# grantjr1842/index-tts

Measured on AMD Instinct MI355X. Metric: synthesised audio seconds per second (IndexTTS-2 infer_v2 hot path), whole job, higher is better.
Workload: dtype f32 (greedy decode + its prefill: exact fp32 MFMA; fp32 accumulate and fp32 activations everywhere) + split-bf16 (fp32 operands as hi+lo bf16, 3 bf16 MFMAs per product) GEMMs, DiT attention and convolutions in s2mel, the latent pass and the vocoder; GPT linear weights STORED as bf16 (rounded once at

## Files before the change

index-tts_amd/csrc/capi.hip:

```cpp
#include <cstring>
#include <new>

#include "../../include/idxtts.h"
#include "bigvgan.h"
#include "cond.h"
#include "semantic.h"
#include "codec.h"
#include "audio.h"
#include "campplus.h"
#include "conv1d.h"
#include "ctx.h"
#include "gpt.h"
#include "model_util.h"
#include "s2mel.h"

namespace idxtts {

static thread_local std::string g_last_error;

void set_error(const std::string& msg) { g_last_error = msg; }
int fail(const char* file, int line, const std::string& msg) {
  const char* base = std::strrchr(file, '/');
  g_last_error = std::string(base ? base + 1 : file) + ":" + std::to_string(line) + ": " + msg;
  return 1;
}

int aa_act_forward(void* y, const void* x, const float* up_f, const float* down_f, const float* log_alpha,
                   const float* log_beta, int B, int C, int T, hipStream_t stream, const int* lens = nullptr, int len_mul = 1, int dtype = 0);

}

using namespace idxtts;

struct idxtts_conv1d {
  ConvWeights w;
  DeviceArena arena;
  int Cout = 0;
};

struct idxtts_linear {
  LinearWeights w;
  DeviceArena arena;
};

#define API_BEGIN try {
#define API_END                                                        \
  }                                                                    \
  catch (const std::exception& e) { return fail(__FILE__, __LINE__, std::string("exception: ") + e.what()); } \
  catch (...) { return fail(__FILE__, __LINE__, "unknown exception"); }

extern "C" {

int idxtts_version(void) { return 100; }

const char* idxtts_last_error(void) { return g_last_error.c_str(); }

int idxtts_aa_act_fwd(void* out, const void* in, const float* up_filter, const float* down_filter,
                      const float* log_alpha, const float* log_beta, int B, int C, int T, int dtype, void* stream) {
  API_BEGIN
  IDX_CHECK(dtype == IDXTTS_DTYPE_F32 || dtype == IDXTTS_DTYPE_F16 || dtype == IDXTTS_DTYPE_BF16, "dtype must be IDXTTS_DTYPE_F32 / F16 / BF16");
  IDX_CHECK(B >= 0 && C >= 0 && T >= 0, "negative shape");
  return aa_act_forward(out, in, up_filter, down_filter, log_alpha, log_beta, B, C, T, static_cast<hipStream_t>(stream), nullptr, 1, dtype);
  API_END
}

static int fetch(const float* src, size_t n, std::vector<float>* dst) {
  dst->resize(n);
  if (!n) return 0;
  const hipError_t e = hipMemcpy(dst->data(), src, n * sizeof(float), hipMemcpyDefault);
  if (e == hipErrorNoDevice) {
    (void)hipGetLastError();
    memcpy(dst->data(), src, n * sizeof(float));
    return 0;
  }
  IDX_HIP(e);
  return 0;
}

int idxtts_conv1d_create(const float* weight, const float* bias, int Cout, int Cin, int K, int transposed_stride,
                         idxtts_conv1d** out) {
  API_BEGIN
  IDX_CHECK(weight && out, "null pointer");
  IDX_CHECK(Cout > 0 && Cin > 0 && K > 0 && transposed_stride >= 1, "bad shape");
  std::unique_ptr<idxtts_conv1d> c(new idxtts_conv1d());
  std::vector<float> hw, hb;
  if (fetch(weight, (size_t)Cout * Cin * K, &hw)) return 1;
  c->Cout = Cout;
  c->w.Cin = Cin;
  c->w.nchunk = cdiv(Cin, CONV_KC);
  c->w.ups = transposed_stride;
  if (transposed_stride > 1) {
    IDX_CHECK(K == 2 * transposed_stride, "ConvTranspose1d kernel must be 2*stride");
    c->w.M = Cout * transposed_stride;
    c->w.K = 3;
  } else {
    c->w.M = Cout;
    c->w.K = K;
  }
  std::vector<float> packed(conv_packed_floats(c->w.M, Cin, c->w.K));
  if (transposed_stride > 1) pack_conv_transpose1d(packed.data(), hw.data(), Cin, Cout, K, transposed_stride);
  else pack_conv1d(packed.data(), hw.data(), Cout, Cin, K);
  float* d = nullptr;
  if (c->arena.upload(packed.data(), packed.size(), &d)) return 1;
  c->w.wp = d;
  {
    std::vector<float> p16(packed.size());
    pack_conv_bf16x3(p16.data(), packed.data(), packed.size() / CONV_SUB);
    if (c->arena.upload(p16.data(), p16.size(), &d)) return 1;
    c->w.wp16 = d;
  }
  if (bias) {
    if (fetch(bias, Cout, &hb)) return 1;
    if (c->arena.upload(hb.data(), hb.size(), &d)) return 1;
    c->w.bias = d;
  }
  *out = c.release();
  return 0;
  API_END
}

int idxtts_conv1d_fwd(const idxtts_conv1d* conv, const float* x, float* y, const float* residual, int B, int T,
                      int dilation, int pad_left, int pad_mode, float scale, int accumulate, void* stream) {
  API_BEGIN
  IDX_CHECK(conv, "null handle");
  if (B == 0 || T == 0) return 0;
  ConvArgs a;
  a.x = x; a.y = y; a.res = residual; a.B = B; a.T = T; a.dil = dilation; a.pad_left = pad_left;
  a.pad_mode = pad_mode; a.scale = scale; a.accum = accumulate;
  return conv1d_forward(conv->w, a, static_cast<hipStream_t>(stream));
  API_END
}

int idxtts_conv1d_destroy(idxtts_conv1d* conv) {
  delete conv;
  return 0;
}

int idxtts_ctx_load_tensor(idxtts_ctx* ctx, const char* name, const float* data, const int64_t* shape, int ndim) {
  API_BEGIN
  IDX_CHECK(ctx && name && shape, "null pointer");
  IDX_CHECK(!ctx->finalized, "context already finalized");
  IDX_CHECK(ndim >= 0 && ndim <= 8, "ndim");
  const std::string key(name);
  if (!ctx->model->accepts(key)) IDX_FAIL("unknown tensor name '" + key + "'");
  HostTensor t;
  t.shape.assign(shape, shape + ndim);
  const int64_t n = t.numel();
  IDX_CHECK(n >= 0, "negative numel");
  IDX_CHECK(n == 0 || data, "null data");
  if (fetch(data, (size_t)n, &t.data)) return 1;
  ctx->tensors[key] = std::move(t);
  return 0;
  API_END
}

int idxtts_ctx_finalize(idxtts_ctx* ctx) {
  API_BEGIN
  IDX_CHECK(ctx, "null ctx");
  IDX_CHECK(!ctx->finalized, "context already finalized");
  if (ctx->model->finalize(ctx->tensors, ctx->arena)) return 1;
  ctx->tensors.clear();
  ctx->finalized = true;
  return 0;
  API_END
}

int idxtts_ctx_get_tensor(idxtts_ctx* ctx, const char* name, float* host_out, size_t capacity) {
  API_BEGIN
  IDX_CHECK(ctx && name && host_out, "null pointer");
  IDX_CHECK(!ctx->finalized, "staged tensors are released by finalize");
  auto it = ctx->tensors.find(name);
  if (it == ctx->tensors.end()) IDX_FAIL(std::string("no staged tensor '") + name + "'");
  IDX_CHECK(capacity >= it->second.data.size(), "output buffer too small");
  std::copy(it->second.data.begin(), it->second.data.end(), host_out);
  return 0;
  API_END
}

int idxtts_ctx_destroy(idxtts_ctx* ctx) {
  delete ctx;
  return 0;
}

float idxtts_fp8_e4m3_decode(unsigned char code) { return fp8_e4m3_decode(code); }
unsigned char idxtts_fp8_e4m3_encode(float v) { return fp8_e4m3_encode(v); }

int idxtts_bigvgan_create(const idxtts_bigvgan_config* cfg, idxtts_ctx** out) {
  API_BEGIN
  IDX_CHECK(cfg && out, "null pointer");
  std::unique_ptr<idxtts_ctx> ctx(new idxtts_ctx());
  ctx->model.reset(new BigVGANModel(*cfg));
  *out = ctx.release();
  return 0;
  API_END
}

size_t idxtts_bigvgan_workspace_bytes(const idxtts_ctx* ctx, int B, int Tm) {
  if (!ctx || B <= 0 || Tm <= 0) return 0;
  auto* m = dynamic_cast<const BigVGANModel*>(ctx->model.get());
  return m ? m->workspace_bytes(B, Tm) : 0;
}

int idxtts_bigvgan_fwd(idxtts_ctx* ctx, const float* mel, float* wav, int B, int Tm, void* workspace,
                       size_t workspace_bytes, int clamp, int stage_idx, float* stage_out, void* stream) {
  API_BEGIN
  IDX_CHECK(ctx, "null ctx");
  IDX_CHECK(ctx->finalized, "context not finalized");
  auto* m = dynamic_cast<BigVGANModel*>(ctx->model.get());
  IDX_CHECK(m, "not a BigVGAN context");
  IDX_CHECK(B >= 0 && Tm >= 0, "negative shape");
  return m->forward(mel, wav, B, Tm, workspace, workspace_bytes, clamp, stage_idx, stage_out, static_cast<hipStream_t>(stream));
  API_END
}

int idxtts_bigvgan_fwd_ragged(idxtts_ctx* ctx, const float* mel, const int* mel_lengths, float* wav, int B, int Tm, void* workspace,
                              size_t workspace_bytes, int clamp, void* stream) {
  API_BEGIN
  IDX_CHECK(ctx && ctx->finalized, "context not finalized");
  auto* m = dynamic_cast<BigVGANModel*>(ctx->model.get());
  IDX_CHECK(m, "not a BigVGAN context");
  IDX_CHECK(B >= 0 && Tm >= 0 && mel_lengths, "shape / lengths");
  return m->forward(mel, wav, B, Tm, workspace, workspace_bytes, clamp, 0, nullptr, static_cast<hipStream_t>(stream), mel_lengths);
  API_END
}


int idxtts_linear_create(const float* weight, const float* bias, int N, int K, int weight_is_kn, idxtts_linear** out) {
  API_BEGIN
  IDX_CHECK(weight && out && N > 0 && K > 0, "bad arguments");
  std::unique_ptr<idxtts_linear> l(new idxtts_linear());
  std::vector<float> hw, hb;
  if (fetch(weight, (size_t)N * K, &hw)) return 1;
  if (bias && fetch(bias, N, &hb)) return 1;
  if (make_linear(l->arena, hw.data(), bias ? hb.data() : nullptr, N, K, {WP16_ALWAYS, weight_is_kn ? W_KN : W_NK}, &l->w)) return 1;
  *out = l.release();
  return 0;
  API_END
}

int idxtts_linear_fwd(const idxtts_linear* lin, const float* x, int ldx, float* y, int ldy, const float* residual, int ldr, int M,
                      int act, int bf16x3, void* stream) {
  API_BEGIN
  IDX_CHECK(lin, "null handle");
  GemmArgs a;
  a.x = x; a.ldx = ldx; a.y = y; a.ldy = ldy; a.res = residual; a.ldr = ldr; a.M = M; a.act = act;
  return bf16x3 ? gemm_bf16x3_forward(lin->w, a, static_cast<hipStream_t>(stream)) : gemm_tn_forward(lin->w, a, static_cast<hipStream_t>(stream));
  API_END
}

int idxtts_linear_destroy(idxtts_linear* lin) {
  delete lin;
  return 0;
}

int idxtts_attention_fwd(const float* q, const float* k, const float* v, float* o, long q_batch_stride, int q_token_stride,
                         long kv_batch_stride, int kv_token_stride, long o_batch_stride, int o_token_stride, int B, int H,
                         int Sq, int Sk, int causal, const int* kstart, const int* kend, float scale, void* stream) {
  API_BEGIN
  AttnArgs a;
  a.q = q; a.k = k; a.v = v; a.o = o;
  a.q_bs = q_batch_stride; a.k_bs = a.v_bs = kv_batch_stride; a.o_bs = o_batch_stride;
  a.q_ts = q_token_stride; a.k_ts = a.v_ts = kv_token_stride; a.o_ts = o_token_stride;
  a.B = B; a.H = H; a.Sq = Sq; a.Sk = Sk; a.causal = causal; a.kstart = kstart; a.kend = kend; a.scale = scale;
  return flash_attn_forward(a, static_cast<hipStream_t>(stream));
  API_END
}

int idxtts_attention_relkey_fwd(const float* q, const float* k, const float* v, float* o, long batch_stride, int token_stride,
                                long o_batch_stride, int o_token_stride, int B, int H, int S, const int* kend, float scale,
                                const float* rel_key, int rel_left, int rel_right, int split_bf16, void* stream) {
  API_BEGIN
  IDX_CHECK(rel_key, "rel_key is null");
  AttnArgs a;
  a.q = q; a.k = k; a.v = v; a.o = o;
  a.q_bs = a.k_bs = a.v_bs = batch_stride; a.o_bs = o_batch_stride;
  a.q_ts = a.k_ts = a.v_ts = token_stride; a.o_ts = o_token_stride;
  a.B = B; a.H = H; a.Sq = S; a.Sk = S; a.causal = 0; a.kend = kend; a.scale = scale;
  a.rel_key = rel_key; a.rel_left = rel_left; a.rel_right = rel_right; a.split_bf16 = split_bf16 ? 1 : 0;
  return flash_attn_forward(a, static_cast<hipStream_t>(stream));
  API_END
}

int idxtts_attention_bf16x3_fwd(const float* q, const float* k, const float* v, float* o, long q_batch_stride, int q_token_stride,
                         long kv_batch_stride, int kv_token_stride, long o_batch_stride, int o_token_stride, int B, int H,
                         int Sq, int Sk, int causal, const int* kstart, const int* kend, float scale, void* stream) {
  API_BEGIN
  AttnArgs a;
  a.q = q; a.k = k; a.v = v; a.o = o;
  a.q_bs = q_batch_stride; a.k_bs = a.v_bs = kv_batch_stride; a.o_bs = o_batch_stride;
  a.q_ts = q_token_stride; a.k_ts = a.v_ts = kv_token_stride; a.o_ts = o_token_stride;
  a.B = B; a.H = H; a.Sq = Sq; a.Sk = Sk; a.causal = causal; a.kstart = kstart; a.kend = kend; a.scale = scale; a.split_bf16 = 1;
  return flash_attn_forward(a, static_cast<hipStream_t>(stream));
  API_END
}

int idxtts_layernorm_fwd(const float* x, float* y, const float* gamma, const float* beta, int M, int d, float eps, void* stream) {
  API_BEGIN
  RowsNormArgs n;
  n.x_in = x; n.ld_in = d; n.y = y; n.ld_y = d; n.M = M; n.d = d; n.mode = NORM_LN; n.eps = eps; n.g1 = gamma; n.b1 = beta;
  return rows_norm_forward(n, static_cast<hipStream_t>(stream));
  API_END
}

int idxtts_gpt_create(const idxtts_gpt_config* cfg, idxtts_ctx** out) {
  API_BEGIN
  IDX_CHECK(cfg && out, "null pointer");
  std::unique_ptr<idxtts_ctx> ctx(new idxtts_ctx());
  ctx->model.reset(new GPTModel(*cfg));
  *out = ctx.release();
  return 0;
  API_END
}

int idxtts_gpt_quantize_weights(idxtts_ctx* ctx, int format) {
  API_BEGIN
  IDX_CHECK(ctx, "null ctx");
  IDX_CHECK(!ctx->finalized, "quantise before idxtts_ctx_finalize");
  auto* m = dynamic_cast<GPTModel*>(ctx->model.get());
  IDX_CHECK(m, "not a GPT context");
  return m->quantize_weights(ctx->tensors, format);
  API_END
}

int idxtts_gpt_set_kv_format(idxtts_ctx* ctx, int format) {
  API_BEGIN
  IDX_CHECK(ctx, "null ctx");
  IDX_CHECK(format == 0 || format == 1, "KV cache format: 0 (fp32) or 1 (bf16)");
  auto* m = dynamic_cast<GPTModel*>(ctx->model.get());
  IDX_CHECK(m, "not a GPT context");
  IDX_CHECK(m->kv_fmt == format || m->generating.load() == 0, "a generation is in flight on this context: switch the KV format between generations");
  m->kv_fmt = format;
  return 0;
  API_END
}

int idxtts_gpt_get_kv_format(const idxtts_ctx* ctx) {
  if (!ctx) return -1;
  auto* m = dynamic_cast<const GPTModel*>(ctx->model.get());
  return m ? m->kv_fmt : -1;
}

int idxtts_gpt_graph_cache_entries(idxtts_ctx* ctx) {
  if (!ctx || !ctx->finalized) return -1;
  auto* m = dynamic_cast<GPTModel*>(ctx->model.get());
  if (!m) return -1;
  std::lock_guard<std::mutex> l(m->graph_mu);
  return (int)m->graph_cache.size();
}

size_t idxtts_gpt_workspace_bytes(const idxtts_ctx* ctx, int B, int S, int max_new_tokens) {
  if (!ctx || B <= 0 || S <= 0 || max_new_tokens < 0 || !ctx->finalized) return 0;
  auto* m = dynamic_cast<const GPTModel*>(ctx->model.get());
  return m ? m->workspace_bytes(B, S, max_new_tokens) : 0;
}

#define GPT_MODEL(ctx)                                        \
  IDX_CHECK(ctx, "null ctx");                                 \
  IDX_CHECK(ctx->finalized, "context not finalized");         \
  auto* m = dynamic_cast<GPTModel*>(ctx->model.get());        \
  IDX_CHECK(m, "not a GPT context")

int idxtts_gpt_embed(idxtts_ctx* ctx, float* out, int rows, const int* text_ids, const int* text_pos_idx, const int* mel_ids,
                     const int* mel_pos_idx, const float* extra, const int* extra_idx, void* stream) {
  API_BEGIN
  GPT_MODEL(ctx);
  return m->embed(out, rows, text_ids, text_pos_idx, mel_ids, mel_pos_idx, extra, extra_idx, static_cast<hipStream_t>(stream));
  API_END
}

int idxtts_gpt_generate(idxtts_ctx* ctx, const float* inputs_embeds, const int* pad_left, int B, int P, int max_new_tokens,
                        float repetition_penalty, long long* codes, int* n_steps, float* logits_out, void* workspace,
                        size_t workspace_bytes, int use_graph, void* stream) {
  API_BEGIN
  GPT_MODEL(ctx);
  return m->generate(inputs_embeds, pad_left, B, P, max_new_tokens, repetition_penalty, nullptr, codes, n_steps, logits_out, workspace,
                     workspace_bytes, use_graph, static_cast<hipStream_t>(stream));
  API_END
}

int idxtts_gpt_generate_forced(idxtts_ctx* ctx, const float* inputs_embeds, const int* pad_left, int B, int P, int max_new_tokens,
                               float repetition_penalty, const long long* forced_codes, long long* codes, int* n_steps, float* logits_out,
                               void* workspace, size_t workspace_bytes, void* stream) {
  API_BEGIN
  GPT_MODEL(ctx);
  IDX_CHECK(forced_codes, "null forced_codes");
  return m->generate(inputs_embeds, pad_left, B, P, max_new_tokens, repetition_penalty, nullptr, codes, n_steps, logits_out, workspace,
                     workspace_bytes, 0, static_cast<hipStream_t>(stream), forced_codes);
  API_END
}

int idxtts_gpt_generate_sampled(idxtts_ctx* ctx, const float* inputs_embeds, const int* pad_left, int B, int P, int max_new_tokens,
                                float repetition_penalty, const idxtts_sampling* sampling, long long* codes, int* n_steps,
                                float* logits_out, void* workspace, size_t workspace_bytes, int use_graph, void* stream) {
  API_BEGIN
  GPT_MODEL(ctx);
  IDX_CHECK(sampling, "null sampling configuration");
  return m->generate(inputs_embeds, pad_left, B, P, max_new_tokens, repetition_penalty, sampling, codes, n_steps, logits_out, workspace,
                     workspace_bytes, use_graph, static_cast<hipStream_t>(stream));
  API_END
}

size_t idxtts_gpt_beam_workspace_bytes(const idxtts_ctx* ctx, int B, int num_beams, int S, int max_new_tokens) {
  if (!ctx || !ctx->finalized || B <= 0 || num_beams < 2 || S <= 0 || max_new_tokens <= 0) return 0;
  auto* m = dynamic_cast<const GPTModel*>(ctx->model.get());
  return m ? m->beam_workspace_bytes(B, num_beams, S, max_new_tokens) : 0;
}

int idxtts_gpt_generate_beam(idxtts_ctx* ctx, const float* inputs_embeds, const int* pad_left, int B, int P, int max_new_tokens,
                             float repetition_penalty, const idxtts_beam* beam, long long* codes, int* n_steps, void* workspace,
                             size_t workspace_bytes, int use_graph, void* stream) {
  API_BEGIN
  GPT_MODEL(ctx);
  return m->generate_beam(inputs_embeds, pad_left, B, P, max_new_tokens, repetition_penalty, beam, codes, n_steps, workspace,
                          workspace_bytes, use_graph, static_cast<hipStream_t>(stream));
  API_END
}

size_t idxtts_gpt_session_workspace_bytes(const idxtts_ctx* ctx, int slots, int max_prompt, int max_new_tokens) {
  if (!ctx || !ctx->finalized || slots <= 0 || slots > 64 || max_prompt <= 0 || max_new_tokens <= 0) return 0;
  auto* m = dynamic_cast<const GPTModel*>(ctx->model.get());
  return m ? m->session_workspace_bytes(slots, max_prompt, max_new_tokens) : 0;
}

int idxtts_gpt_session_init(idxtts_ctx* ctx, int slots, int max_prompt, int max_new_tokens, float repetition_penalty, void* workspace,
                            size_t workspace_bytes, void* stream) {
  API_BEGIN
  GPT_MODEL(ctx);
  return m->session_init(workspace, workspace_bytes, slots, max_prompt, max_new_tokens, repetition_penalty, static_cast<hipStream_t>(stream));
  API_END
}

size_t idxtts_gpt_session_workspace_bytes_ex(const idxtts_ctx* ctx, int slots, int max_prompt, int max_new_tokens, int flags) {
  if (!ctx || !ctx->finalized || slots <= 0 || slots > 64 || max_prompt <= 0 || max_new_tokens <= 0) return 0;
  if (flags & ~IDXTTS_SESSION_SAMPLED) return 0;
  auto* m = dynamic_cast<const GPTModel*>(ctx->model.get());
  return m ? m->session_workspace_bytes(slots, max_prompt, max_new_tokens, (flags & IDXTTS_SESSION_SAMPLED) != 0) : 0;
}

int idxtts_gpt_session_init_ex(idxtts_ctx* ctx, int slots, int max_prompt, int max_new_tokens, float repetition_penalty, int flags,
                               void* workspace, size_t workspace_bytes, void* stream) {
  API_BEGIN
  GPT_MODEL(ctx);
  IDX_CHECK(!(flags & ~IDXTTS_SESSION_SAMPLED), "unknown session flags");
  return m->session_init(workspace, workspace_bytes, slots, max_prompt, max_new_tokens, repetition_penalty, static_cast<hipStream_t>(stream),
                         (flags & IDXTTS_SESSION_SAMPLED) != 0);
  API_END
}

int idxtts_gpt_session_admit(idxtts_ctx* ctx, int n, const float* inputs_embeds, int ld_rows, const int* prompt_lens,
                             const int* slot_ids, const int* max_new_tokens, void* workspace, void* stream) {
  API_BEGIN
  GPT_MODEL(ctx);
  return m->session_admit(workspace, n, inputs_embeds, ld_rows, prompt_lens, slot_ids, max_new_tokens, static_cast<hipStream_t>(stream));
  API_END
}

int idxtts_gpt_session_admit_sampled(idxtts_ctx* ctx, int n, const float* inputs_embeds, int ld_rows, const int* prompt_lens,
                                     const int* slot_ids, const int* max_new_tokens, const idxtts_sampling* per_row, void* workspace,
                                     void* stream) {
  API_BEGIN
  GPT_MODEL(ctx);
  IDX_CHECK(per_row, "null pointer");
  return m->session_admit(workspace, n, inputs_embeds, ld_rows, prompt_lens, slot_ids, max_new_tokens, static_cast<hipStream_t>(stream),
                          per_row);
  API_END
}

size_t idxtts_gpt_session_workspace_bytes_beam(const idxtts_ctx* ctx, int slots, int num_beams, int max_prompt, int max_new_tokens) {
  if (!ctx || !ctx->finalized || slots <= 0 || slots > 64 || max_prompt <= 0 || max_new_tokens <= 0) return 0;
  if (num_beams < 2 || num_beams > BEAM_MAX || slots % num_beams) return 0;
  auto* m = dynamic_cast<const GPTModel*>(ctx->model.get());
  return m ? m->session_workspace_bytes(slots, max_prompt, max_new_tokens, false, num_beams) : 0;
}

int idxtts_gpt_session_init_beam(idxtts_ctx* ctx, int slots, int num_beams, int max_prompt, int max_new_tokens, float repetition_penalty,
                                 void* workspace, size_t workspace_bytes, void* stream) {
  API_BEGIN
  GPT_MODEL(ctx);
  IDX_CHECK(num_beams >= 2 && num_beams <= BEAM_MAX, "2 <= num_beams <= 8");
  return m->session_init(workspace, workspace_bytes, slots, max_prompt, max_new_tokens, repetition_penalty, static_cast<hipStream_t>(stream),
                         false, num_beams);
  API_END
}

int idxtts_gpt_session_admit_beam(idxtts_ctx* ctx, int n, const float* inputs_embeds, int ld_rows, const int* prompt_lens,
                                  const int* group_ids, const int* max_new_tokens, const idxtts_beam* per_request, void* workspace,
                                  void* stream) {
  API_BEGIN
  GPT_MODEL(ctx);
  return m->session_admit_beam(workspace, n, inputs_embeds, ld_rows, prompt_lens, group_ids, max_new_tokens, per_request,
                               static_cast<hipStream_t>(stream));
  API_END
}

int idxtts_gpt_session_step(idxtts_ctx* ctx, int n_steps, int use_graph, int* finished_slots, int* n_finished, void* workspace,
                            void* stream) {
  API_BEGIN
  GPT_MODEL(ctx);
  return m->session_step(workspace, n_steps, use_graph, finished_slots, n_finished, static_cast<hipStream_t>(stream));
  API_END
}

int idxtts_gpt_session_read(idxtts_ctx* ctx, int slot, long long* codes, int* n_codes, void* workspace, void* stream) {
  API_BEGIN
  GPT_MODEL(ctx);
  return m->session_read(workspace, slot, codes, n_codes, static_cast<hipStream_t>(stream));
  API_END
}

int idxtts_gpt_session_release(idxtts_ctx* ctx, void* workspace) {
  API_BEGIN
  GPT_MODEL(ctx);
  return m->session_release(workspace);
  API_END
}

int idxtts_gpt_latent(idxtts_ctx* ctx, const float* emb, const int* pad_left, int B, int S, int mel_start, int M, float* latent,
                      void* workspace, size_t workspace_bytes, void* stream) {
  API_BEGIN
  GPT_MODEL(ctx);
  return m->latent(emb, pad_left, B, S, mel_start, M, latent, workspace, workspace_bytes, static_cast<hipStream_t>(stream));
  API_END
}


int idxtts_cond_create(const idxtts_cond_config* cfg, idxtts_ctx** out) {
  API_BEGIN
  IDX_CHECK(cfg && out, "null pointer");
  std::unique_ptr<idxtts_ctx> ctx(new idxtts_ctx());
  ctx->model.reset(new CondModel(*cfg));
  *out = ctx.release();
  return 0;
  API_END
}

size_t idxtts_cond_workspace_bytes(const idxtts_ctx* ctx, int B, int T) {
  if (!ctx || !ctx->finalized || B <= 0 || T < 3) return 0;
  auto* m = dynamic_cast<const CondModel*>(ctx->model.get());
  return m ? m->workspace_bytes(B, T) : 0;
}

int idxtts_cond_forward(idxtts_ctx* ctx, const float* feats, const int* lengths, int B, int T, float* out, void* workspace,
                        size_t workspace_bytes, void* stream) {
  API_BEGIN
  IDX_CHECK(ctx, "null ctx");
  IDX_CHECK(ctx->finalized, "context not finalized");
  auto* m = dynamic_cast<CondModel*>(ctx->model.get());
  IDX_CHECK(m, "not a conditioning-encoder context");
  return m->forward(feats, lengths, B, T, out, workspace, workspace_bytes, static_cast<hipStream_t>(stream));
  API_END
}

int idxtts_w2vbert_create(const idxtts_w2vbert_config* cfg, idxtts_ctx** out) {
  API_BEGIN
  IDX_CHECK(cfg && out, "null pointer");
  std::unique_ptr<idxtts_ctx> ctx(new idxtts_ctx());
  ctx->model.reset(new W2VBertModel(*cfg));
  *out = ctx.release();
  return 0;
  API_END
}

size_t idxtts_w2vbert_workspace_bytes(const idxtts_ctx* ctx, int B, int T) {
  if (!ctx || !ctx->finalized || B <= 0 || T <= 0) return 0;
  auto* m = dynamic_cast<const W2VBertModel*>(ctx->model.get());
  return m ? m->workspace_bytes(B, T) : 0;
}

int idxtts_w2vbert_forward(idxtts_ctx* ctx, const float* feats, const int* lengths, int B, int T, float* out, void* workspace,
                           size_t workspace_bytes, void* stream) {
  API_BEGIN
  IDX_CHECK(ctx, "null ctx");
  IDX_CHECK(ctx->finalized, "context not finalized");
  auto* m = dynamic_cast<W2VBertModel*>(ctx->model.get());
  IDX_CHECK(m, "not a w2v-bert context");
  return m->forward(feats, lengths, B, T, out, workspace, workspace_bytes, static_cast<hipStream_t>(stream));
  API_END
}

int idxtts_repcodec_create(const idxtts_repcodec_config* cfg, idxtts_ctx** out) {
  API_BEGIN
  IDX_CHECK(cfg && out, "null pointer");
  std::unique_ptr<idxtts_ctx> ctx(new idxtts_ctx());
  ctx->model.reset(new RepCodecModel(*cfg));
  *out = ctx.release();
  return 0;
  API_END
}

size_t idxtts_repcodec_workspace_bytes(const idxtts_ctx* ctx, int B, int T) {
  if (!ctx || !ctx->finalized || B <= 0 || T <= 0) return 0;
  auto* m = dynamic_cast<const RepCodecModel*>(ctx->model.get());
  return m ? m->workspace_bytes(B, T) : 0;
}

int idxtts_repcodec_quantize(idxtts_ctx* ctx, const float* x, int B, int T, long long* indices, float* quantized, void* workspace,
                             size_t workspace_bytes, void* stream) {
  API_BEGIN
  IDX_CHECK(ctx, "null ctx");
  IDX_CHECK(ctx->finalized, "context not finalized");
  auto* m = dynamic_cast<RepCodecModel*>(ctx->model.get());
  IDX_CHECK(m, "not a semantic-codec context");
  return m->quantize(x, B, T, indices, quantized, workspace, workspace_bytes, static_cast<hipStream_t>(stream));
  API_END
}

int idxtts_melspec_create(const idxtts_melspec_config* cfg, idxtts_ctx** out) {
  API_BEGIN
  IDX_CHECK(cfg && out, "null pointer");
  std::unique_ptr<idxtts_ctx> ctx(new idxtts_ctx());
  ctx->model.reset(new MelSpecModel(*cfg));
  *out = ctx.release();
  return 0;
  API_END
}

int idxtts_melspec_frames(const idxtts_ctx* ctx, int n_samples) {
  if (!ctx || n_samples <= 0) return 0;
  auto* m = dynamic_cast<const MelSpecModel*>(ctx->model.get());
  return m ? m->frames(n_samples) : 0;
}

size_t idxtts_melspec_workspace_bytes(const idxtts_ctx* ctx, int B, int n_samples) {
  if (!ctx || !ctx->finalized || B <= 0 || n_samples <= 0) return 0;
  auto* m = dynamic_cast<const MelSpecModel*>(ctx->model.get());
  return m ? m->workspace_bytes(B, n_samples) : 0;
}

int idxtts_melspec_forward(idxtts_ctx* ctx, const float* audio, int B, int n_samples, float* mel, void* workspace, size_t workspace_bytes,
                           void* stream) {
  API_BEGIN
  IDX_CHECK(ctx, "null ctx");
  IDX_CHECK(ctx->finalized, "context not finalized");
  auto* m = dynamic_cast<MelSpecModel*>(ctx->model.get());
  IDX_CHECK(m, "not a mel-spectrogram context");
  return m->forward(audio, B, n_samples, mel, workspace, workspace_bytes, static_cast<hipStream_t>(stream));
  API_END
}

int idxtts_campplus_create(const idxtts_campplus_config* cfg, idxtts_ctx** out) {
  API_BEGIN
  IDX_CHECK(cfg && out, "null pointer");
  std::unique_ptr<idxtts_ctx> ctx(new idxtts_ctx());
  ctx->model.reset(new CamPPlusModel(*cfg));
  *out = ctx.release();
  return 0;
  API_END
}

size_t idxtts_campplus_workspace_bytes(const idxtts_ctx* ctx, int T) {
  if (!ctx || !ctx->finalized || T < 8) return 0;
  auto* m = dynamic_cast<const CamPPlusModel*>(ctx->model.get());
  return m ? m->workspace_bytes(T) : 0;
}

int idxtts_campplus_forward(idxtts_ctx* ctx, const float* feat, int B, int T, float* style, void* workspace, size_t workspace_bytes, void* stream) {
  API_BEGIN
  IDX_CHECK(ctx, "null ctx");
  IDX_CHECK(ctx->finalized, "context not finalized");
  auto* m = dynamic_cast<CamPPlusModel*>(ctx->model.get());
  IDX_CHECK(m, "not a CAMPPlus context");
  return m->forward(feat, B, T, style, workspace, workspace_bytes, static_cast<hipStream_t>(stream));
  API_END
}

int idxtts_emovec_merge(float* out, const float* base, const float* emo, float alpha, size_t n, void* stream) {
  API_BEGIN
  return lerp_rows(out, base, emo, alpha, n, static_cast<hipStream_t>(stream));
  API_END
}

int idxtts_s2mel_create(const idxtts_s2mel_config* cfg, idxtts_ctx** out) {
  API_BEGIN
  IDX_CHECK(cfg && out, "null pointer");
  std::unique_ptr<idxtts_ctx> ctx(new idxtts_ctx());
  ctx->model.reset(new S2MelModel(*cfg));
  *out = ctx.release();
  return 0;
  API_END
}

#define S2MEL_MODEL(ctx)                                      \
  IDX_CHECK(ctx, "null ctx");                                 \
  IDX_CHECK(ctx->finalized, "context not finalized");         \
  auto* m = dynamic_cast<S2MelModel*>(ctx->model.get());      \
  IDX_CHECK(m, "not an s2mel context")

size_t idxtts_s2mel_cond_workspace_bytes(const idxtts_ctx* ctx, int B, int M, int Tg) {
  if (!ctx || !ctx->finalized || B <= 0 || M <= 0 || Tg <= 0) return 0;
  auto* m = dynamic_cast<const S2MelModel*>(ctx->model.get());
  return m ? m->cond_workspace_bytes(B, M, Tg) : 0;
}

int idxtts_s2mel_prepare_cond(idxtts_ctx* ctx, const float* latent, const long long* codes, const int* code_lens,
                              const int* target_lens, int B, int M, int Tg, float* cond_out, void* workspace,
                              size_t workspace_bytes, void* stream) {
  API_BEGIN
  S2MEL_MODEL(ctx);
  return m->prepare_cond(latent, codes, code_lens, target_lens, B, M, Tg, cond_out, workspace, workspace_bytes,
                         static_cast<hipStream_t>(stream));
  API_END
}

int idxtts_s2mel_regulate(idxtts_ctx* ctx, const float* S, const int* in_lens, const int* target_lens, int B, int M, int Tg, float* cond_out,
                          void* workspace, size_t workspace_bytes, void* stream) {
  API_BEGIN
  S2MEL_MODEL(ctx);
  return m->regulate(S, in_lens, target_lens, B, M, Tg, cond_out, workspace, workspace_bytes, static_cast<hipStream_t>(stream));
  API_END
}

size_t idxtts_s2mel_cfm_workspace_bytes(const idxtts_ctx* ctx, int B, int T, int n_steps) {
  if (!ctx || !ctx->finalized || B <= 0 || T <= 0 || n_steps <= 0) return 0;
  auto* m = dynamic_cast<const S2MelModel*>(ctx->model.get());
  return m ? m->cfm_workspace_bytes(B, T, n_steps) : 0;
}

int idxtts_s2mel_cfm(idxtts_ctx* ctx, const float* mu, const int* x_lens, const float* prompt, const int* prompt_lens, int Tp_max,
                     const float* style, const float* z, const float* t_emb, const float* dt, int n_steps, float cfg_rate,
                     float* out, int B, int T, void* workspace, size_t workspace_bytes, void* stream) {
  API_BEGIN
  S2MEL_MODEL(ctx);
  return m->cfm(mu, x_lens, prompt, prompt_lens, Tp_max, style, z, t_emb, dt, n_steps, cfg_rate, out, B, T, workspace,
                workspace_bytes, static_cast<hipStream_t>(stream));
  API_END
}

size_t idxtts_s2mel_cfm_rows_workspace_bytes(const idxtts_ctx* ctx, int B, int T, int Tp_max, int n_steps) {
  if (!ctx || !ctx->finalized || B <= 0 || T <= 0 || Tp_max <= 0 || n_steps <= 0) return 0;
  auto* m = dynamic_cast<const S2MelModel*>(ctx->model.get());
  return m ? m->cfm_rows_workspace_bytes(B, T, Tp_max, n_steps) : 0;
}

int idxtts_s2mel_cfm_rows(idxtts_ctx* ctx, const float* gen_cond, const int* target_lens, int Tg_max, const float* const* prompt_conditions,
                          const float* const* ref_mels, const int* prompt_lens, const float* style, const float* z, const float* t_emb,
                          const float* dt, int n_steps, float cfg_rate, float* out, int B, int T, void* workspace, size_t workspace_bytes,
                          void* stream) {
  API_BEGIN
  S2MEL_MODEL(ctx);
  return m->cfm_rows(gen_cond, target_lens, Tg_max, prompt_conditions, ref_mels, prompt_lens, style, z, t_emb, dt, n_steps, cfg_rate, out,
                     B, T, workspace, workspace_bytes, static_cast<hipStream_t>(stream));
  API_END
}

int idxtts_s2mel_estimator(idxtts_ctx* ctx, const float* x, const float* prompt, const int* prompt_lens, int Tp_max, const int* x_lens,
                           const float* t_emb, const float* style, const float* mu, float* out, int B, int T, void* workspace,
                           size_t workspace_bytes, void* stream) {
  API_BEGIN
  S2MEL_MODEL(ctx);
  return m->estimator(x, prompt, prompt_lens, Tp_max, x_lens, t_emb, style, mu, out, B, T, workspace, workspace_bytes,
                      static_cast<hipStream_t>(stream));
  API_END
}


int idxtts_set_gemm_mode(int mode) {
  set_gemm_mode(mode);
  return 0;
}

int idxtts_get_gemm_mode(void) { return get_gemm_mode(); }

int idxtts_set_decode_geometry(int narrow) {
  set_decode_geometry(narrow);
  return 0;
}

int idxtts_get_decode_geometry(void) { return get_decode_geometry(); }

int idxtts_release_stream(void* stream) {
  API_BEGIN
  hipStream_t st = static_cast<hipStream_t>(stream);
  return gemm_release_stream_scratch(st) || s2mel_release_stream(st);
  API_END
}

int idxtts_set_decode_plane_rows(int min_rows) {
  API_BEGIN
  IDX_CHECK(min_rows == 0 || (min_rows >= 5 && min_rows <= 65), "0 (default), 5..64 or 65 (off)");
  set_decode_plane_rows(min_rows);
  return 0;
  API_END
}

int idxtts_get_decode_plane_rows(void) { return get_decode_plane_rows(); }

int idxtts_s2mel_set_overlap(int on) {
  set_s2mel_overlap(on);
  return 0;
}

int idxtts_s2mel_get_overlap(void) { return get_s2mel_overlap(); }

}
```

index-tts_amd/csrc/gemm.h:

```cpp
#pragma once
#include "common.h"

namespace idxtts {

enum GemmAct { ACT_NONE = 0, ACT_GELU_NEW = 1, ACT_SILU = 2, ACT_SWIGLU = 3, ACT_MISH = 4, ACT_GATE = 5 ,
               ACT_GELU_ERF = 6 , ACT_RELU = 7  };

struct LinearWeights {
  const float* wp = nullptr;
  const float* bias = nullptr;
  int N = 0, K = 0;
  const void* wp16 = nullptr;
};

static inline size_t linear_packed_floats(int N, int K) { return (size_t)cdiv(N, 32) * cdiv(K, 16) * 512; }

void pack_linear(float* dst, const float* w, int N, int K);

struct GemmArgs {
  const float* x = nullptr; int ldx = 0;
  float* y = nullptr; int ldy = 0;
  const void* x_planes = nullptr;
  void* y_planes = nullptr;
  const float* rope = nullptr; int rope_T = 0, rope_cols = 0;
  const float* res = nullptr; int ldr = 0;
  int M = 0;
  int act = ACT_NONE;
  float out_scale = 1.0f;
  int taps = 1, seq_len = 0, dil = 1, pad_left = 0, pad_mode = 0;
  const int* row_len = nullptr;
  int ksplit = 1;
};

int gemm_tn_forward(const LinearWeights& w, const GemmArgs& a, hipStream_t stream);
int gemm_bf16x3_forward(const LinearWeights& w, const GemmArgs& a, hipStream_t stream);
size_t linear_bf16x3_packed_bytes(int N, int K);
void pack_linear_bf16x3(void* dst, const float* w, int N, int K);

enum GemmMode { GEMM_F32 = 0, GEMM_BF16X3 = 1 };
void set_gemm_mode(int mode);
int get_gemm_mode();
int gemm_forward(const LinearWeights& w, const GemmArgs& a, hipStream_t stream);
bool gemm_uses_planes(const LinearWeights& w, const GemmArgs& a);

int gemm_release_stream_scratch(hipStream_t stream);

}
```

index-tts_amd/csrc/gemm_bf16x3_v2.hip:

```cpp
#include <algorithm>
#include <cstdlib>
#include <cstring>

#include "gemm_common.h"
#include "prof.h"

namespace idxtts {

typedef __bf16 bf16x8 __attribute__((ext_vector_type(8)));
typedef __bf16 bf16x4 __attribute__((ext_vector_type(4)));

size_t linear_planes_bytes(int N, int K) { return (size_t)2 * cdiv(K, 16) * (cdiv(N, 256) * 256) * 16 * sizeof(uint16_t); }

void pack_linear_planes(void* dst, const float* w, int N, int K) {
  uint16_t* o = static_cast<uint16_t*>(dst);
  const int KC = cdiv(K, 16), NP = cdiv(N, 256) * 256;
  std::memset(o, 0, linear_planes_bytes(N, K));
  uint16_t* lo = o + (size_t)KC * NP * 16;
  for (int n = 0; n < N; ++n)
    for (int k = 0; k < K; ++k) {
      const float x = w[(size_t)n * K + k];
      const uint16_t hi = f2bf(x);
      const size_t idx = ((size_t)(k >> 4) * NP + n) * 16 + (k & 15);
      o[idx] = hi;
      lo[idx] = f2bf(x - bf2f(hi));
    }
}

__global__ __launch_bounds__(256) void split_planes_kernel(const float* __restrict__ x, int ldx, int M, int K, __bf16* __restrict__ hi,
                                                           __bf16* __restrict__ lo) {
  const int k = blockIdx.y * 64 + (threadIdx.x & 15) * 4;
#pragma unroll
  for (int i = 0; i < 4; ++i) {
    const int m = blockIdx.x * 64 + (threadIdx.x >> 4) + 16 * i;
    if (m >= M || k >= ((K + 15) & ~15)) continue;
    const f32x4 v = k < K ? *reinterpret_cast<const f32x4*>(x + (size_t)m * ldx + k) : f32x4{0.f, 0.f, 0.f, 0.f};
    bf16x4 h, l;
    split_bf16_x4(v, h, l);
    const size_t o = ((size_t)(k >> 4) * M + m) * 16 + (k & 15);
    *reinterpret_cast<bf16x4*>(hi + o) = h;
    *reinterpret_cast<bf16x4*>(lo + o) = l;
  }
}

#ifdef V2_TIMING
static unsigned long long* g_v2_stamps = nullptr;
extern "C" int idxtts_dbg_v2_stamps(void* buf) { g_v2_stamps = static_cast<unsigned long long*>(buf); return 0; }
#define V2_STAMP(k) do { if (q.stamps && tid == 64) q.stamps[(size_t)blockIdx.x * 8 + (k)] = __builtin_amdgcn_s_memtime(); } while (0)
#define V2_RSTAMP(k) do { if (q.stamps && tid == 64) q.stamps[(size_t)blockIdx.x * 8 + (k)] = __builtin_amdgcn_s_memrealtime(); } while (0)
#else
#define V2_STAMP(k)
#define V2_RSTAMP(k)
#endif

struct GemmV2P {
  GemmKP g;
  const __bf16* a_hi; const __bf16* a_lo;
  const __bf16* b_hi; const __bf16* b_lo;
  int a_rows, npad, nstages;
  int a_bytes, b_bytes;
  int a_plane, b_plane;
  int cs, nbg;
#ifdef V2_TIMING
  unsigned long long* stamps;
#endif
};

struct V2Rsrc { __amdgpu_buffer_rsrc_t a, b; };

#define V2_WAITCNT(vm) __builtin_amdgcn_s_waitcnt(((vm) & 15) | (((vm) >> 4) << 14) | 0x70)

template <bool TAPS, int EPI, int CFG>
__device__ __forceinline__ void gemm_v2_tile(const GemmV2P& q, const int bm, const int bn, const int tid) {
  constexpr int NSTAGE = CFG ? 3 : 4;
  constexpr int WMW = CFG ? 2 : 4, WNW = 2, TN = CFG ? 2 : 4;
  constexpr int BM = 64 * WMW, BN = 32 * TN * WNW;
  static_assert(BM / 32 == WMW * WNW && BN / 32 == WMW * WNW, "one 32-row block of A and of B per wave and plane");
  constexpr int PLANE = BM * 32;
  constexpr int STAGE_BYTES = 4 * PLANE;
  constexpr int PPW = 4;
  const GemmKP& p = q.g;
  extern __shared__ __attribute__((aligned(1024))) char smv2[];

  const int wave = __builtin_amdgcn_readfirstlane(tid >> 6), lane = tid & 63;
  const int h = lane >> 5, j = lane & 31;
  const int wm = wave >> 1, wn = wave & 1;

  const int lrow = lane >> 1;
  const int dunit = (lane & 1) ^ ((lrow >> 3) & 1);
  const int a_m = bm * BM + 32 * wave + lrow;
  const __amdgpu_buffer_rsrc_t rA = __builtin_amdgcn_make_buffer_rsrc(const_cast<__bf16*>(q.a_hi), 0, q.a_bytes, 0x00020000);
  const __amdgpu_buffer_rsrc_t rB = __builtin_amdgcn_make_buffer_rsrc(const_cast<__bf16*>(q.b_hi), 0, q.b_bytes, 0x00020000);
  const int voffB = (bn * BN + 32 * wave + lrow) * 32 + dunit * 16;
  int voffA = min(a_m, q.a_rows - 1) * 32 + dunit * 16;
  int seq_base = 0, seq_t = 0, seq_n = 0;
  if (TAPS) {
    const int sb = a_m / p.seq_len;
    seq_base = sb * p.seq_len;
    seq_t = a_m - seq_base;
    seq_n = (p.row_len && a_m < p.M) ? min(p.row_len[sb], p.seq_len) : p.seq_len;
  }
  auto tap_voff = [&](int tap) -> int {
    int t = seq_t + tap * p.dil - p.pad_left;
    if (p.pad_mode == 1) { t = t < 0 ? -t : t; t = t >= seq_n ? 2 * (seq_n - 1) - t : t; }
    const bool ok = a_m < p.M && t >= 0 && t < seq_n;
    return ok ? (seq_base + t) * 32 + dunit * 16 : (int)0x80000000;
  };
  V2_STAMP(0); V2_RSTAMP(4);
  const int ns = q.nstages;
  const int sA = q.a_rows * 32, sB = q.npad * 32;
  const int cpt = TAPS ? (p.kc >> 4) : ns;
  int ist = 0, soA = 0, soB = 0, ich = 0, itap = 0, wslot = 0, rslot = 0;
  if (TAPS) voffA = tap_voff(0);
  char* const lds_w = smv2 + wave * 1024;
  auto issue_piece = [&](int pi) {
    auto dst = (__attribute__((address_space(3))) void*)(lds_w + wslot * STAGE_BYTES + pi * PLANE);
    if (pi == 0) __builtin_amdgcn_raw_ptr_buffer_load_lds(rA, dst, 16, voffA, soA, 0, 0);
    else if (pi == 1) __builtin_amdgcn_raw_ptr_buffer_load_lds(rA, dst, 16, voffA, soA + q.a_plane, 0, 0);
    else if (pi == 2) __builtin_amdgcn_raw_ptr_buffer_load_lds(rB, dst, 16, voffB, soB, 0, 0);
    else __builtin_amdgcn_raw_ptr_buffer_load_lds(rB, dst, 16, voffB, soB + q.b_plane, 0, 0);
  };
  auto advance = [&]() {
    ++ist;
    wslot = wslot + 1 == NSTAGE ? 0 : wslot + 1;
    soB += sB;
    soA += sA;
    if (TAPS) {
      if (++ich == cpt) { ich = 0; soA = 0; ++itap; voffA = tap_voff(itap); }
    }
  };

  const int sw = (h ^ ((j >> 3) & 1)) * 16;
  const int a_off = (wm * 64 + j) * 32 + sw;
  const int b_offr = (wn * TN * 32 + j) * 32 + sw;

  f32x16 acc[2][TN];
#pragma unroll
  for (int a = 0; a < 2; ++a)
#pragma unroll
    for (int b = 0; b < TN; ++b)
#pragma unroll
      for (int r = 0; r < 16; ++r) acc[a][b][r] = 0.0f;

  for (int s = 0; s < NSTAGE; ++s)
    if (s < ns) {
#pragma unroll
      for (int pi = 0; pi < PPW; ++pi) issue_piece(pi);
      advance();
    }

  struct Frag { bf16x8 ah[2], al[2], bh[TN], bl[TN]; };
  auto wait_stage = [&](int s) {
    const int rem = ns - 1 - s;
    if (NSTAGE >= 4 && rem >= 2) V2_WAITCNT(2 * PPW);
    else if (NSTAGE >= 3 && rem >= 1) V2_WAITCNT(PPW);
    else V2_WAITCNT(0);
    __builtin_amdgcn_s_barrier();
    __builtin_amdgcn_sched_barrier(0);
  };
  auto load_frags = [&](Frag& f) {
    const char* st = smv2 + rslot * STAGE_BYTES;
    rslot = rslot + 1 == NSTAGE ? 0 : rslot + 1;
#pragma unroll
    for (int t = 0; t < 2; ++t) {
      f.ah[t] = *reinterpret_cast<const bf16x8*>(st + a_off + t * 1024);
      f.al[t] = *reinterpret_cast<const bf16x8*>(st + PLANE + a_off + t * 1024);
    }
#pragma unroll
    for (int t = 0; t < TN; ++t) {
      f.bh[t] = *reinterpret_cast<const bf16x8*>(st + 2 * PLANE + b_offr + t * 1024);
      f.bl[t] = *reinterpret_cast<const bf16x8*>(st + 3 * PLANE + b_offr + t * 1024);
    }
  };
  auto compute = [&](const Frag& f, const bool more) {
#define V2_MFMA3(mt, nt)                                                                                         \
    acc[mt][nt] = __builtin_amdgcn_mfma_f32_32x32x16_bf16(f.al[mt], f.bh[nt], acc[mt][nt], 0, 0, 0);             \
    acc[mt][nt] = __builtin_amdgcn_mfma_f32_32x32x16_bf16(f.ah[mt], f.bl[nt], acc[mt][nt], 0, 0, 0);             \
    acc[mt][nt] = __builtin_amdgcn_mfma_f32_32x32x16_bf16(f.ah[mt], f.bh[nt], acc[mt][nt], 0, 0, 0);
    if constexpr (TN == 4) { V2_MFMA3(0, 0) V2_MFMA3(0, 1) } else { V2_MFMA3(0, 0) }
    __builtin_amdgcn_sched_barrier(0);
    if (more) issue_piece(0);
    __builtin_amdgcn_sched_barrier(0);
    if constexpr (TN == 4) { V2_MFMA3(0, 2) V2_MFMA3(0, 3) } else { V2_MFMA3(0, 1) }
    __builtin_amdgcn_sched_barrier(0);
    if (more) issue_piece(1);
    __builtin_amdgcn_sched_barrier(0);
    if constexpr (TN == 4) { V2_MFMA3(1, 0) V2_MFMA3(1, 1) } else { V2_MFMA3(1, 0) }
    __builtin_amdgcn_sched_barrier(0);
    if (more) issue_piece(2);
    __builtin_amdgcn_sched_barrier(0);
    if constexpr (TN == 4) { V2_MFMA3(1, 2) V2_MFMA3(1, 3) } else { V2_MFMA3(1, 1) }
    __builtin_amdgcn_sched_barrier(0);
    if (more) { issue_piece(3); advance(); }
    __builtin_amdgcn_sched_barrier(0);
#undef V2_MFMA3
  };

  Frag f0, f1;
  {
    const int rem = ns - 1;
    if (NSTAGE >= 4 && rem >= 3) V2_WAITCNT(3 * PPW);
    else if (NSTAGE >= 3 && rem >= 2) V2_WAITCNT(2 * PPW);
    else if (rem >= 1) V2_WAITCNT(PPW);
    else V2_WAITCNT(0);
    __builtin_amdgcn_s_barrier();
    __builtin_amdgcn_sched_barrier(0);
  }
  V2_STAMP(1);
  load_frags(f0);
  int i = 0;
  for (; i + NSTAGE + 1 < ns; i += 2) {
    V2_WAITCNT((NSTAGE - 2) * PPW);
    __builtin_amdgcn_s_barrier();
    __builtin_amdgcn_sched_barrier(0);
    load_frags(f1);
    compute(f0, true);
    V2_WAITCNT((NSTAGE - 2) * PPW);
    __builtin_amdgcn_s_barrier();
    __builtin_amdgcn_sched_barrier(0);
    load_frags(f0);
    compute(f1, true);
  }
  for (; i < ns; i += 2) {
    if (i + 1 < ns) { wait_stage(i + 1); load_frags(f1); }
    else V2_WAITCNT(0);
    compute(f0, ist < ns);
    if (i + 1 < ns) {
      if (i + 2 < ns) { wait_stage(i + 2); load_frags(f0); }
      else V2_WAITCNT(0);
      compute(f1, ist < ns);
    }
  }
  V2_STAMP(2);
  auto write_pass = [&](int ps, float* lds, int RS) {
    const int mt = ps >> 1, hh = ps & 1;
#pragma unroll
    for (int nt = 0; nt < TN; ++nt)
#pragma unroll
      for (int qq = 0; qq < 2; ++qq)
#pragma unroll
        for (int e = 0; e < 4; ++e) lds[(8 * qq + 4 * h + e) * RS + nt * 32 + j] = acc[mt][nt][(2 * hh + qq) * 4 + e];
  };
  gemm_epilogue_wave<EPI, TN, 3>(p, write_pass, reinterpret_cast<float*>(smv2), bm * BM + wm * 64, bn * BN + wn * TN * 32, wave, lane);
  V2_STAMP(6);
#ifdef V2_TIMING
  asm volatile("s_waitcnt vmcnt(0)" ::: "memory");
#endif
  V2_STAMP(3); V2_RSTAMP(5);
}

template <bool TAPS, int EPI, int CFG>
__global__ __launch_bounds__(CFG ? 256 : 512, CFG ? 3 : 2) void gemm_bf16x3_v2_kernel(const GemmV2P q) {
  const GemmKP& p = q.g;
  const int L = blockIdx.x, xcd = L & 7, qq = L >> 3;
  int bn, bm;
  if (p.n_fast) {
    const int cs = q.cs, cg = xcd % cs, rc = xcd / cs;
    const int bml = qq / q.nbg, bnl = qq - bml * q.nbg;
    bm = bml * (8 / cs) + rc;
    bn = cg * q.nbg + bnl;
    if (bn >= p.nblocks) return;
  } else { bn = qq / p.mt8; bm = (qq - bn * p.mt8) * 8 + xcd; }
  if (bm >= p.mtiles) return;
  gemm_v2_tile<TAPS, EPI, CFG>(q, bm, bn, threadIdx.x);
}

StreamScratch g_plane_scratch(8);

int gemm_bf16x3_v2_forward(GemmKP p, const void* wplanes, const LinearWeights& w, const GemmArgs& a, hipStream_t stream, double flops,
                           double bytes) {
  IDX_CHECK(w.K % 16 == 0 && (a.taps <= 1 || (w.K / a.taps) % 16 == 0), "v2 needs K % 16 == 0");
  const int xk = a.taps > 1 ? w.K / a.taps : w.K;
  const size_t plane = (size_t)(xk / 16) * a.M * 16 * sizeof(__bf16);
  void* scratch = nullptr;
  if (!a.x_planes && g_plane_scratch.acquire(stream, 2 * plane, &scratch)) return 1;
  const __bf16* hi = static_cast<const __bf16*>(a.x_planes ? a.x_planes : scratch);
  const __bf16* lo = hi + plane / sizeof(__bf16);
  if (!a.x_planes) {
    static const int cat_split = prof_register("split_planes_kernel");
    ProfScope prof(cat_split, stream, 0.0, 8.0 * a.M * (double)xk);
    hipLaunchKernelGGL(split_planes_kernel, dim3(cdiv(a.M, 64), cdiv(xk, 64)), dim3(256), 0, stream, a.x, a.ldx, a.M, xk, const_cast<__bf16*>(hi), const_cast<__bf16*>(lo));
    IDX_LAUNCH_CHECK();
  }
  GemmV2P q;
  q.g = p;
  if (a.y_planes) {
    const int n_out = (a.act == ACT_SWIGLU || a.act == ACT_GATE) ? w.N / 2 : w.N;
    IDX_CHECK(n_out % 16 == 0 && (a.ldy & 3) == 0, "output planes need N_out % 16 == 0");
    q.g.y_hi = static_cast<__bf16*>(a.y_planes);
    q.g.y_lo = q.g.y_hi + plane_elems(a.M, n_out);
  }
  if (a.rope) {
    IDX_CHECK(a.rope_T > 0 && a.rope_cols % 64 == 0 && a.act == ACT_NONE && (a.ldy & 3) == 0, "fused rotary arguments");
    q.g.rope = a.rope; q.g.rope_T = a.rope_T; q.g.rope_cols = a.rope_cols;
  }
  const int cfg = 1;
  const int BMh = cfg ? 128 : 256, BNh = cfg ? 128 : 256;
  q.g.mtiles = cdiv(a.M, BMh);
  q.g.mt8 = cdiv(q.g.mtiles, 8);
  q.g.nblocks = cdiv(w.N, BNh);
  q.a_hi = hi; q.a_lo = lo; q.a_rows = a.M;
  q.npad = cdiv(w.N, 256) * 256;
  q.b_hi = static_cast<const __bf16*>(wplanes);
  q.b_lo = q.b_hi + (size_t)(w.K / 16) * q.npad * 16;
  q.nstages = w.K / 16;
#ifdef V2_TIMING
  q.stamps = g_v2_stamps;
#endif
  const size_t b_plane = (size_t)(w.K / 16) * q.npad * 32;
  IDX_CHECK(2 * plane < (1ull << 31) && 2 * b_plane < (1ull << 31), "operand planes beyond the 2 GiB a buffer offset addresses");
  q.a_plane = (int)plane; q.a_bytes = (int)(2 * plane);
  q.b_plane = (int)b_plane; q.b_bytes = (int)(2 * b_plane);
  q.cs = 1;
  static const double cs_bytes = [] { const char* e = getenv("IDXTTS_GEMM_CS_BYTES"); return e ? atof(e) : 3.2e6; }();
  if (!q.g.n_fast && (double)w.N * w.K * 4.0 <= 8.0 * cs_bytes && a.M > w.N) q.g.n_fast = 1;
  if (q.g.n_fast) {
    while (q.cs < 8 && (double)w.N * w.K * 4.0 / q.cs > cs_bytes && q.g.nblocks >= 2 * q.cs) q.cs *= 2;
  }
  q.nbg = cdiv(q.g.nblocks, q.cs);
  const int64_t grid = q.g.n_fast ? (int64_t)8 * q.nbg * cdiv(q.g.mtiles, 8 / q.cs) : (int64_t)8 * q.g.nblocks * q.g.mt8;
  IDX_CHECK(grid < (1ll << 31), "grid size");
  static const int cat = prof_register("gemm_bf16x3_v2_kernel");
  ProfScope prof(cat, stream, flops, bytes);
  const int lds = cfg ? 3 * (4 * 128 * 32) : 4 * (4 * 256 * 32);
  const bool paired = a.act == ACT_SWIGLU || a.act == ACT_GATE;
  IDX_CHECK(!(a.rope && (a.res || paired)), "the rotary epilogue takes no residual and no paired activation");
  IDX_CHECK(!a.row_len || a.seq_len >= 16, "row masks need seq_len >= 16");
  const int epi = a.rope ? EPI_ROPE : paired ? EPI_PAIRED : a.act != ACT_NONE ? EPI_ACT : EPI_PLAIN;
  typedef void (*KernelFn)(const GemmV2P);
#define V2_ROW(T, C) gemm_bf16x3_v2_kernel<T, EPI_PLAIN, C>, gemm_bf16x3_v2_kernel<T, EPI_ROPE, C>, gemm_bf16x3_v2_kernel<T, EPI_PAIRED, C>, gemm_bf16x3_v2_kernel<T, EPI_ACT, C>
  static const KernelFn kernels[2][2][4] = {{{V2_ROW(false, 0)}, {V2_ROW(true, 0)}}, {{V2_ROW(false, 1)}, {V2_ROW(true, 1)}}};
  static DynLdsLimit lds_limit[2];
  IDX_HIP(lds_limit[0].set(4 * (4 * 256 * 32), V2_ROW(false, 0), V2_ROW(true, 0)));
  IDX_HIP(lds_limit[1].set(3 * (4 * 128 * 32), V2_ROW(false, 1), V2_ROW(true, 1)));
#undef V2_ROW
  hipLaunchKernelGGL(kernels[cfg][a.taps > 1 ? 1 : 0][epi], dim3((unsigned)grid), dim3(cfg ? 256 : 512), lds, stream, q);
  IDX_LAUNCH_CHECK();
  return 0;
}

}
```

index-tts_amd/csrc/model_util.h:

```cpp
#pragma once
#include <map>
#include <string>
#include <vector>

#include "ctx.h"
#include "gemm.h"

namespace idxtts {

int need(std::map<std::string, HostTensor>& t, const std::string& key, std::vector<int64_t> shape, HostTensor** out);
int up(DeviceArena& arena, const std::vector<float>& v, const float** out);
int tensor_from(std::map<std::string, HostTensor>& t, DeviceArena& arena, const std::string& key, std::vector<int64_t> shape, const float** out);
int vec_from(std::map<std::string, HostTensor>& t, DeviceArena& arena, const std::string& key, int n, const float** out);
int ln_from(std::map<std::string, HostTensor>& t, DeviceArena& arena, const std::string& prefix, int n, const float** g, const float** b);

enum Wp16Policy {
  WP16_ALWAYS,
  WP16_DMA_SHAPES,
};
enum WeightLayout { W_NK , W_KN  };
struct LinearOpts {
  Wp16Policy wp16;
  WeightLayout layout = W_NK;
  int Kpad = 0;
};
int make_linear(DeviceArena& arena, const float* w, const float* bias, int N, int K, const LinearOpts& o, LinearWeights* out);
int linear_from(std::map<std::string, HostTensor>& t, DeviceArena& arena, const std::string& prefix, int N, int K, bool bias, Wp16Policy wp16,
                LinearWeights* out, std::vector<int64_t> wshape = {});

struct Carver {
  char* base; size_t off = 0;
  explicit Carver(void* b) : base(static_cast<char*>(b)) {}
  template <typename T> T* take(size_t n) {
    off = (off + 255) & ~(size_t)255;
    T* p = base ? reinterpret_cast<T*>(base + off) : nullptr;
    off += n * sizeof(T);
    return p;
  }
};

int lin(const LinearWeights& w, const float* x, int ldx, float* y, int ldy, int M, hipStream_t st, int act = ACT_NONE,
        const float* res = nullptr, int ldr = 0);
int lin_exact(const LinearWeights& w, const float* x, int ldx, float* y, int ldy, int M, hipStream_t st, int act = ACT_NONE,
              const float* res = nullptr, int ldr = 0);
int layer_norm(const float* x, float* y, const float* g, const float* b, int M, int d, hipStream_t st);

}
```

index-tts_amd/csrc/model_util.hip:

```cpp
#include "model_util.h"

#include <cstring>

#include "norm.h"

namespace idxtts {

int need(std::map<std::string, HostTensor>& t, const std::string& key, std::vector<int64_t> shape, HostTensor** out) {
  auto it = t.find(key);
  if (it == t.end()) IDX_FAIL("missing tensor '" + key + "'");
  if (it->second.shape != shape) {
    std::string s = "tensor '" + key + "' has shape [";
    for (auto d : it->second.shape) s += std::to_string(d) + ",";
    s += "] expected [";
    for (auto d : shape) s += std::to_string(d) + ",";
    IDX_FAIL(s + "]");
  }
  *out = &it->second;
  return 0;
}

int up(DeviceArena& arena, const std::vector<float>& v, const float** out) {
  float* d = nullptr;
  if (arena.upload(v.data(), v.size(), &d)) return 1;
  *out = d;
  return 0;
}

int tensor_from(std::map<std::string, HostTensor>& t, DeviceArena& arena, const std::string& key, std::vector<int64_t> shape, const float** out) {
  HostTensor* h = nullptr;
  if (need(t, key, shape, &h)) return 1;
  return up(arena, h->data, out);
}

int vec_from(std::map<std::string, HostTensor>& t, DeviceArena& arena, const std::string& key, int n, const float** out) {
  return tensor_from(t, arena, key, {n}, out);
}

int ln_from(std::map<std::string, HostTensor>& t, DeviceArena& arena, const std::string& prefix, int n, const float** g, const float** b) {
  return vec_from(t, arena, prefix + ".weight", n, g) || vec_from(t, arena, prefix + ".bias", n, b);
}

int make_linear(DeviceArena& arena, const float* w, const float* bias, int N, int K, const LinearOpts& o, LinearWeights* out) {
  const int Kpad = o.Kpad ? o.Kpad : K;
  IDX_CHECK(Kpad >= K, "Kpad < K");
  std::vector<float> rows;
  if (o.layout == W_KN || Kpad != K) {
    rows.assign((size_t)N * Kpad, 0.0f);
    for (int n = 0; n < N; ++n)
      for (int k = 0; k < K; ++k) rows[(size_t)n * Kpad + k] = o.layout == W_KN ? w[(size_t)k * N + n] : w[(size_t)n * K + k];
    w = rows.data();
  }
  std::vector<float> packed(linear_packed_floats(N, Kpad));
  pack_linear(packed.data(), w, N, Kpad);
  if (up(arena, packed, &out->wp)) return 1;
  out->N = N; out->K = Kpad;
  if (o.wp16 == WP16_ALWAYS || (N >= 96 && Kpad % 16 == 0)) {
    std::vector<float> p16((linear_bf16x3_packed_bytes(N, Kpad) + 3) / 4);
    pack_linear_bf16x3(p16.data(), w, N, Kpad);
    const float* d16 = nullptr;
    if (up(arena, p16, &d16)) return 1;
    out->wp16 = d16;
  }
  if (bias && up(arena, std::vector<float>(bias, bias + N), &out->bias)) return 1;
  return 0;
}

int linear_from(std::map<std::string, HostTensor>& t, DeviceArena& arena, const std::string& prefix, int N, int K, bool bias, Wp16Policy wp16,
                LinearWeights* out, std::vector<int64_t> wshape) {
  HostTensor *w = nullptr, *b = nullptr;
  if (wshape.empty()) wshape = {N, K};
  if (need(t, prefix + ".weight", wshape, &w)) return 1;
  if (bias && need(t, prefix + ".bias", {N}, &b)) return 1;
  return make_linear(arena, w->data.data(), b ? b->data.data() : nullptr, N, K, {wp16, W_NK, (K + 3) & ~3}, out);
}

static GemmArgs lin_args(const float* x, int ldx, float* y, int ldy, int M, int act, const float* res, int ldr) {
  GemmArgs g;
  g.x = x; g.ldx = ldx; g.y = y; g.ldy = ldy; g.M = M; g.act = act; g.res = res; g.ldr = ldr;
  return g;
}

int lin(const LinearWeights& w, const float* x, int ldx, float* y, int ldy, int M, hipStream_t st, int act, const float* res, int ldr) {
  const GemmArgs g = lin_args(x, ldx, y, ldy, M, act, res, ldr);
  if (act == ACT_GELU_ERF || act == ACT_RELU) return gemm_tn_forward(w, g, st);
  return gemm_forward(w, g, st);
}

int lin_exact(const LinearWeights& w, const float* x, int ldx, float* y, int ldy, int M, hipStream_t st, int act, const float* res, int ldr) {
  return gemm_tn_forward(w, lin_args(x, ldx, y, ldy, M, act, res, ldr), st);
}

int layer_norm(const float* x, float* y, const float* g, const float* b, int M, int d, hipStream_t st) {
  RowsNormArgs n;
  n.x_in = x; n.ld_in = d; n.y = y; n.ld_y = d; n.M = M; n.d = d; n.mode = NORM_LN; n.eps = 1e-5f; n.g1 = g; n.b1 = b;
  return rows_norm_forward(n, st);
}

}
```

index-tts_amd/csrc/s2mel.hip:

```cpp
#include <cmath>
#include <cstring>

#include <map>
#include <mutex>
#include <utility>

#include "model_util.h"
#include "s2mel.h"

namespace idxtts {

S2MelModel::S2MelModel(const idxtts_s2mel_config& c) : cfg(c) {}

bool S2MelModel::accepts(const std::string& name) const {
  static const char* prefixes[] = {"cfm.estimator.", "length_regulator.", "gpt_layer.", "semantic_codec.", "rope_cache"};
  for (const char* p : prefixes)
    if (name.rfind(p, 0) == 0) return true;
  return false;
}

namespace {

std::vector<float> col_slice(const std::vector<float>& w, int N, int K, int k0, int k1) {
  std::vector<float> o((size_t)N * (k1 - k0));
  for (int n = 0; n < N; ++n) std::memcpy(&o[(size_t)n * (k1 - k0)], &w[(size_t)n * K + k0], (k1 - k0) * sizeof(float));
  return o;
}

std::vector<float> pair_pack(const float* a, const float* b, int H, int K) {
  std::vector<float> o((size_t)2 * H * K);
  for (int blk = 0; blk < H / 32; ++blk) {
    std::memcpy(&o[(size_t)(blk * 64) * K], a + (size_t)blk * 32 * K, (size_t)32 * K * sizeof(float));
    std::memcpy(&o[(size_t)(blk * 64 + 32) * K], b + (size_t)blk * 32 * K, (size_t)32 * K * sizeof(float));
  }
  return o;
}

std::vector<float> conv_to_rows(const std::vector<float>& w, int Cout, int Cin, int k) {
  std::vector<float> o((size_t)Cout * Cin * k);
  for (int co = 0; co < Cout; ++co)
    for (int ci = 0; ci < Cin; ++ci)
      for (int kk = 0; kk < k; ++kk) o[((size_t)co * k + kk) * Cin + ci] = w[((size_t)co * Cin + ci) * k + kk];
  return o;
}

}

int S2MelModel::finalize(std::map<std::string, HostTensor>& t, DeviceArena& arena) {
  const int D = cfg.hidden_dim, C = cfg.in_channels, Wh = cfg.wn_hidden, depth = cfg.depth;
  IDX_CHECK(D == cfg.num_heads * 64, "head_dim must be 64");
  IDX_CHECK(Wh == D, "the reference's FinalLayer requires wavenet.hidden_dim == DiT.hidden_dim");
  IDX_CHECK((D & 31) == 0 && (Wh & 31) == 0 && (cfg.lr_channels & 31) == 0, "channel counts must be multiples of 32");
  {
    const int nh = (int)(2 * (4 * D) / 3);
    ffn = (nh % 256 == 0) ? nh : nh + 256 - (nh % 256);
  }
  const std::string e = "cfm.estimator";
  blocks.resize(depth);
  std::vector<float> mod_w, mod_b;
  auto append_mod = [&](const std::string& name) -> int {
    HostTensor *w = nullptr, *b = nullptr;
    if (need(t, name + ".project_layer.weight", {2 * D, D}, &w) || need(t, name + ".project_layer.bias", {2 * D}, &b)) return 1;
    mod_w.insert(mod_w.end(), w->data.begin(), w->data.end());
    mod_b.insert(mod_b.end(), b->data.begin(), b->data.end());
    return 0;
  };
  for (int i = 0; i < depth; ++i) {
    DiTBlock& B = blocks[i];
    const std::string p = e + ".transformer.layers." + std::to_string(i);
    if (linear_from(t, arena, p + ".attention.wqkv", 3 * D, D, false, WP16_ALWAYS, &B.wqkv)) return 1;
    if (linear_from(t, arena, p + ".attention.wo", D, D, false, WP16_ALWAYS, &B.wo)) return 1;
    HostTensor *w1 = nullptr, *w3 = nullptr;
    if (need(t, p + ".feed_forward.w1.weight", {ffn, D}, &w1) || need(t, p + ".feed_forward.w3.weight", {ffn, D}, &w3)) return 1;
    if (make_linear(arena, pair_pack(w1->data.data(), w3->data.data(), ffn, D).data(), nullptr, 2 * ffn, D, {WP16_ALWAYS}, &B.w13)) return 1;
    if (linear_from(t, arena, p + ".feed_forward.w2", D, ffn, false, WP16_ALWAYS, &B.w2)) return 1;
    HostTensor *g = nullptr;
    if (need(t, p + ".attention_norm.norm.weight", {D}, &g) || up(arena, g->data, &B.attn_g)) return 1;
    if (need(t, p + ".ffn_norm.norm.weight", {D}, &g) || up(arena, g->data, &B.ffn_g)) return 1;
    if (append_mod(p + ".attention_norm") || append_mod(p + ".ffn_norm")) return 1;
    if (i > depth / 2) {
      HostTensor *sw = nullptr, *sb = nullptr;
      if (need(t, p + ".skip_in_linear.weight", {D, 2 * D}, &sw) || need(t, p + ".skip_in_linear.bias", {D}, &sb)) return 1;
      if (make_linear(arena, col_slice(sw->data, D, 2 * D, 0, D).data(), sb->data.data(), D, D, {WP16_ALWAYS}, &B.skip_a)) return 1;
      if (make_linear(arena, col_slice(sw->data, D, 2 * D, D, 2 * D).data(), nullptr, D, D, {WP16_ALWAYS}, &B.skip_b)) return 1;
    }
  }
  {
    HostTensor* g = nullptr;
    if (need(t, e + ".transformer.norm.norm.weight", {D}, &g) || up(arena, g->data, &final_g)) return 1;
    if (append_mod(e + ".transformer.norm")) return 1;
    if (make_linear(arena, mod_w.data(), mod_b.data(), (2 * depth + 1) * 2 * D, D, {WP16_ALWAYS}, &mod_all)) return 1;
  }
  const int Win = 2 * C + D + cfg.style_dim;
  if (linear_from(t, arena, e + ".cond_projection", D, cfg.content_dim, true, WP16_ALWAYS, &cond_proj)) return 1;
  if (linear_from(t, arena, e + ".cond_x_merge_linear", D, Win, true, WP16_ALWAYS, &merge)) return 1;
  if (linear_from(t, arena, e + ".t_embedder.mlp.0", D, 256, true, WP16_ALWAYS, &temb0) || linear_from(t, arena, e + ".t_embedder.mlp.2", D, D, true, WP16_ALWAYS, &temb2)) return 1;
  if (linear_from(t, arena, e + ".t_embedder2.mlp.0", Wh, 256, true, WP16_ALWAYS, &t2emb0) || linear_from(t, arena, e + ".t_embedder2.mlp.2", Wh, Wh, true, WP16_ALWAYS, &t2emb2)) return 1;
  {
    HostTensor *sw = nullptr, *sb = nullptr;
    if (need(t, e + ".skip_linear.weight", {D, D + C}, &sw) || need(t, e + ".skip_linear.bias", {D}, &sb)) return 1;
    if (make_linear(arena, col_slice(sw->data, D, D + C, 0, D).data(), sb->data.data(), D, D, {WP16_ALWAYS}, &skiplin_a)) return 1;
    if (make_linear(arena, col_slice(sw->data, D, D + C, D, D + C).data(), nullptr, D, C, {WP16_ALWAYS}, &skiplin_b)) return 1;
  }
  if (linear_from(t, arena, e + ".conv1", Wh, D, true, WP16_ALWAYS, &conv1)) return 1;
  if (linear_from(t, arena, e + ".res_projection", Wh, D, true, WP16_ALWAYS, &res_proj)) return 1;
  if (linear_from(t, arena, e + ".final_layer.linear", Wh, Wh, true, WP16_ALWAYS, &final_lin)) return 1;
  if (linear_from(t, arena, e + ".final_layer.adaLN_modulation.1", 2 * Wh, Wh, true, WP16_ALWAYS, &final_mod)) return 1;
  {
    HostTensor *w = nullptr, *b = nullptr;
    if (need(t, e + ".conv2.weight", {C, Wh, 1}, &w) || need(t, e + ".conv2.bias", {C}, &b)) return 1;
    if (make_linear(arena, w->data.data(), b->data.data(), C, Wh, {WP16_ALWAYS}, &conv2)) return 1;
  }
  const int L = cfg.wn_layers, k = cfg.wn_kernel;
  wn.resize(L);
  {
    HostTensor *cw = nullptr, *cb = nullptr;
    if (need(t, e + ".wavenet.cond_layer.conv.conv.weight", {2 * Wh * L, Wh, 1}, &cw) ||
        need(t, e + ".wavenet.cond_layer.conv.conv.bias", {2 * Wh * L}, &cb)) return 1;
    std::vector<float> cw_perm, cb_perm;
    for (int l = 0; l < L; ++l) {
      WNLayer& W = wn[l];
      const std::string p = e + ".wavenet.in_layers." + std::to_string(l) + ".conv.conv";
      HostTensor *iw = nullptr, *ib = nullptr;
      if (need(t, p + ".weight", {2 * Wh, Wh, k}, &iw) || need(t, p + ".bias", {2 * Wh}, &ib)) return 1;
      const std::vector<float> rows = conv_to_rows(iw->data, 2 * Wh, Wh, k);
      if (make_linear(arena, pair_pack(rows.data(), rows.data() + (size_t)Wh * k * Wh, Wh, k * Wh).data(), nullptr, 2 * Wh, k * Wh, {WP16_ALWAYS}, &W.in_gate)) return 1;
      const float* cwl = cw->data.data() + (size_t)l * 2 * Wh * Wh;
      const std::vector<float> cwp = pair_pack(cwl, cwl + (size_t)Wh * Wh, Wh, Wh);
      cw_perm.insert(cw_perm.end(), cwp.begin(), cwp.end());
      std::vector<float> bsum(2 * Wh);
      for (int c = 0; c < 2 * Wh; ++c) bsum[c] = cb->data[(size_t)l * 2 * Wh + c] + ib->data[c];
      const std::vector<float> bp = pair_pack(bsum.data(), bsum.data() + Wh, Wh, 1);
      cb_perm.insert(cb_perm.end(), bp.begin(), bp.end());
      const std::string r = e + ".wavenet.res_skip_layers." + std::to_string(l) + ".conv.conv";
      const int rc = l < L - 1 ? 2 * Wh : Wh;
      HostTensor *rw = nullptr, *rb = nullptr;
      if (need(t, r + ".weight", {rc, Wh, 1}, &rw) || need(t, r + ".bias", {rc}, &rb)) return 1;
      if (l < L - 1) {
        std::vector<float> w_res(rw->data.begin(), rw->data.begin() + (size_t)Wh * Wh), b_res(rb->data.begin(), rb->data.begin() + Wh);
        std::vector<float> w_skip(rw->data.begin() + (size_t)Wh * Wh, rw->data.end()), b_skip(rb->data.begin() + Wh, rb->data.end());
        if (make_linear(arena, w_res.data(), b_res.data(), Wh, Wh, {WP16_ALWAYS}, &W.res) || make_linear(arena, w_skip.data(), b_skip.data(), Wh, Wh, {WP16_ALWAYS}, &W.skip)) return 1;
      } else {
        W.has_res = false;
        if (make_linear(arena, rw->data.data(), rb->data.data(), Wh, Wh, {WP16_ALWAYS}, &W.skip)) return 1;
      }
    }
    if (make_linear(arena, cw_perm.data(), cb_perm.data(), 2 * Wh * L, Wh, {WP16_ALWAYS}, &wn_cond)) return 1;
  }
  const int LC = cfg.lr_channels;
  if (linear_from(t, arena, "length_regulator.content_in_proj", LC, cfg.lr_in_channels, true, WP16_ALWAYS, &lr_in)) return 1;
  lr_conv.resize(cfg.lr_num_convs);
  lr_gn_g.resize(cfg.lr_num_convs);
  lr_gn_b.resize(cfg.lr_num_convs);
  for (int n = 0; n < cfg.lr_num_convs; ++n) {
    HostTensor *w = nullptr, *b = nullptr, *g = nullptr, *bb = nullptr;
    const std::string p = "length_regulator.model." + std::to_string(3 * n);
    if (need(t, p + ".weight", {LC, LC, 3}, &w) || need(t, p + ".bias", {LC}, &b)) return 1;
    if (make_linear(arena, conv_to_rows(w->data, LC, LC, 3).data(), b->data.data(), LC, 3 * LC, {WP16_ALWAYS}, &lr_conv[n])) return 1;
    const std::string q = "length_regulator.model." + std::to_string(3 * n + 1);
    if (need(t, q + ".weight", {LC}, &g) || need(t, q + ".bias", {LC}, &bb)) return 1;
    if (up(arena, g->data, &lr_gn_g[n]) || up(arena, bb->data, &lr_gn_b[n])) return 1;
  }
  {
    HostTensor *w = nullptr, *b = nullptr;
    const std::string p = "length_regulator.model." + std::to_string(3 * cfg.lr_num_convs);
    if (need(t, p + ".weight", {LC, LC, 1}, &w) || need(t, p + ".bias", {LC}, &b)) return 1;
    if (make_linear(arena, w->data.data(), b->data.data(), LC, LC, {WP16_ALWAYS}, &lr_out)) return 1;
  }
  {
    const int dims[4] = {cfg.gpt_dim, cfg.gpt_layer_dims[0], cfg.gpt_layer_dims[1], cfg.gpt_layer_dims[2]};
    for (int n = 0; n < 3; ++n)
      if (linear_from(t, arena, "gpt_layer." + std::to_string(n), dims[n + 1], dims[n], true, WP16_ALWAYS, &gl[n])) return 1;
    IDX_CHECK(dims[3] == cfg.codec_hidden && cfg.codec_hidden == cfg.lr_in_channels, "gpt_layer / codec / length-regulator widths");
  }
  {
    HostTensor *cb = nullptr, *ow = nullptr, *ob = nullptr;
    const std::string q = "semantic_codec.quantizer.quantizers.0";
    if (need(t, q + ".codebook.weight", {cfg.codebook_size, cfg.codebook_dim}, &cb) ||
        need(t, q + ".out_project.weight", {cfg.codec_hidden, cfg.codebook_dim, 1}, &ow) ||
        need(t, q + ".out_project.bias", {cfg.codec_hidden}, &ob)) return 1;
    std::vector<float> table((size_t)cfg.codebook_size * cfg.codec_hidden);
    for (int v = 0; v < cfg.codebook_size; ++v)
      for (int h = 0; h < cfg.codec_hidden; ++h) {
        float acc = 0.0f;
        for (int c = 0; c < cfg.codebook_dim; ++c) acc = std::fmaf(cb->data[(size_t)v * cfg.codebook_dim + c], ow->data[(size_t)h * cfg.codebook_dim + c], acc);
        table[(size_t)v * cfg.codec_hidden + h] = acc + ob->data[h];
      }
    if (up(arena, table, &vq_table)) return 1;
  }
  {
    auto it = t.find("rope_cache");
    if (it == t.end()) IDX_FAIL("missing tensor 'rope_cache' ([T][32][2] cos/sin table, precompute_freqs_cis)");
    IDX_CHECK(it->second.shape.size() == 3 && it->second.shape[1] == 32 && it->second.shape[2] == 2, "rope_cache must be [T][32][2]");
    rope_len = (int)it->second.shape[0];
    if (up(arena, it->second.data, &rope)) return 1;
  }
  return 0;
}

struct CfmBuffers {
  float *x_in, *ha, *hb, *hmid, *hn, *qkv, *att, *ff, *xres, *wn_x, *wn_acts, *wn_out, *vout, *condp, *xstate;
  void *hn_p, *att_p, *ff_p, *acts_p;
  void *h_p, *wnx_p, *xres_p;
  std::vector<void*> skips_p;
  std::vector<float*> skips;
  float *t1, *t1s, *mods, *fmod, *t2, *wnb, *tmp_steps;
  int *lens2, *plen, *lens2t;
  int tail_t0 = 0;
  size_t bytes;
};

static CfmBuffers carve_cfm(const S2MelModel& m, void* ws, int B, int T, int n_steps) {
  const auto& c = m.cfg;
  const int D = c.hidden_dim, C = c.in_channels, Wh = c.wn_hidden;
  const size_t M2 = (size_t)2 * B * T;
  const int Win = 2 * C + D + c.style_dim;
  CfmBuffers b;
  Carver k(ws);
  b.x_in = k.take<float>(M2 * Win);
  b.ha = k.take<float>(M2 * D);
  b.hb = k.take<float>(M2 * D);
  b.hmid = k.take<float>(M2 * D);
  b.hn = k.take<float>(M2 * D);
  b.qkv = k.take<float>(M2 * 3 * D);
  b.att = k.take<float>(M2 * D);
  b.ff = k.take<float>(M2 * m.ffn);
  b.xres = k.take<float>(M2 * D);
  b.hn_p = k.take<float>(M2 * std::max(D, Wh));
  b.att_p = k.take<float>(M2 * D);
  b.ff_p = k.take<float>(M2 * m.ffn);
  b.acts_p = k.take<float>(M2 * Wh);
  b.h_p = k.take<float>(M2 * D);
  b.wnx_p = k.take<float>(M2 * Wh);
  b.xres_p = k.take<float>(M2 * D);
  b.wn_x = k.take<float>(M2 * Wh);
  b.wn_acts = k.take<float>(M2 * Wh);
  b.wn_out = k.take<float>(M2 * Wh);
  b.vout = k.take<float>(M2 * C);
  b.condp = k.take<float>((size_t)B * T * D);
  b.xstate = k.take<float>((size_t)B * C * T);
  for (int i = 0; i < c.depth / 2; ++i) b.skips.push_back(k.take<float>(M2 * D));
  for (int i = 0; i < c.depth / 2; ++i) b.skips_p.push_back(k.take<float>(M2 * D));
  b.t1 = k.take<float>((size_t)n_steps * D);
  b.t1s = k.take<float>((size_t)n_steps * D);
  b.tmp_steps = k.take<float>((size_t)n_steps * std::max(D, Wh));
  b.mods = k.take<float>((size_t)n_steps * (2 * c.depth + 1) * 2 * D);
  b.fmod = k.take<float>((size_t)n_steps * 2 * Wh);
  b.t2 = k.take<float>((size_t)n_steps * Wh);
  b.wnb = k.take<float>((size_t)n_steps * c.wn_layers * 2 * Wh);
  b.lens2 = k.take<int>(2 * B);
  b.plen = k.take<int>(B);
  b.lens2t = k.take<int>(2 * B);
  b.bytes = (k.off + 255) & ~(size_t)255;
  return b;
}

size_t S2MelModel::cfm_workspace_bytes(int B, int T, int n_steps) const { return carve_cfm(*this, nullptr, B, T, n_steps).bytes; }

static CfmBuffers half_view(const S2MelModel& m, const CfmBuffers& w, int h, int B, int T) {
  const auto& c = m.cfg;
  const int D = c.hidden_dim, C = c.in_channels, Wh = c.wn_hidden, Win = 2 * C + D + c.style_dim;
  const size_t R = (size_t)h * B * T;
  CfmBuffers v = w;
  auto sh = [&](float* p, int cols) { return p + R * cols; };
  auto shp = [&](void* p, int cols) -> void* { return static_cast<float*>(p) + R * cols; };
  v.x_in = sh(w.x_in, Win); v.ha = sh(w.ha, D); v.hb = sh(w.hb, D); v.hmid = sh(w.hmid, D); v.hn = sh(w.hn, D); v.qkv = sh(w.qkv, 3 * D);
  v.att = sh(w.att, D); v.ff = sh(w.ff, m.ffn); v.xres = sh(w.xres, D); v.wn_x = sh(w.wn_x, Wh); v.wn_acts = sh(w.wn_acts, Wh);
  v.wn_out = sh(w.wn_out, Wh); v.vout = sh(w.vout, C);
  v.hn_p = shp(w.hn_p, std::max(D, Wh)); v.att_p = shp(w.att_p, D); v.ff_p = shp(w.ff_p, m.ffn); v.acts_p = shp(w.acts_p, Wh);
  v.h_p = shp(w.h_p, D); v.wnx_p = shp(w.wnx_p, Wh); v.xres_p = shp(w.xres_p, D);
  for (size_t i = 0; i < w.skips.size(); ++i) { v.skips[i] = sh(w.skips[i], D); v.skips_p[i] = shp(w.skips_p[i], D); }
  v.lens2 = w.lens2 + h * B; v.lens2t = w.lens2t + h * B;
  return v;
}

static int gemm(const LinearWeights& w, const float* x, int ldx, float* y, int ldy, int M, hipStream_t st, int act = ACT_NONE,
                const float* res = nullptr, int ldr = 0, const void* xp = nullptr, void* yp = nullptr) {
  GemmArgs a;
  a.x = xp ? nullptr : x; a.ldx = ldx; a.y = y; a.ldy = ldy; a.M = M; a.act = act; a.res = res; a.ldr = ldr;
  a.x_planes = xp; a.y_planes = yp;
  return gemm_forward(w, a, st);
}

static int dit_eval(S2MelModel& m, CfmBuffers& w, int N2, int T, int step, hipStream_t st, hipEvent_t lag_event) {
  const auto& c = m.cfg;
  const int D = c.hidden_dim, C = c.in_channels, Wh = c.wn_hidden, depth = c.depth, half = depth / 2;
  const int M = N2 * T, Win = 2 * C + D + c.style_dim;
  const float* mods = w.mods + (size_t)step * (2 * depth + 1) * 2 * D;
  bool chain = true;
  {
    GemmArgs pr;
    pr.M = M;
    const LinearWeights* used[] = {&m.blocks[0].wqkv, &m.blocks[0].wo, &m.blocks[0].w13, &m.blocks[0].w2, &m.skiplin_a, &m.final_lin,
                                   &m.wn[0].skip};
    for (const LinearWeights* lw : used) chain = chain && gemm_uses_planes(*lw, pr);
  }
  bool chain_wn = chain;
  {
    GemmArgs pr;
    pr.M = M;
    const LinearWeights* used[] = {&m.skiplin_b, &m.conv1, &m.res_proj, &m.wn[0].res};
    for (const LinearWeights* lw : used) chain_wn = chain_wn && gemm_uses_planes(*lw, pr);
    pr.taps = c.wn_kernel; pr.seq_len = T;
    chain_wn = chain_wn && gemm_uses_planes(m.wn[0].in_gate, pr);
  }
  void* const hn_p = chain ? w.hn_p : nullptr;
  const int t0 = w.tail_t0, Tt = T - t0, Mt = N2 * Tt;
  bool chain_t = chain, chain_wn_t = chain_wn;
  if (t0 > 0) {
    GemmArgs pr;
    pr.M = Mt;
    const LinearWeights* used[] = {&m.blocks[0].wo, &m.blocks[0].w13, &m.blocks[0].w2, &m.skiplin_a, &m.final_lin, &m.wn[0].skip};
    for (const LinearWeights* lw : used) chain_t = chain_t && gemm_uses_planes(*lw, pr);
    chain_wn_t = chain_t && chain_wn && gemm_uses_planes(m.skiplin_b, pr) && gemm_uses_planes(m.conv1, pr) && gemm_uses_planes(m.res_proj, pr) &&
                 gemm_uses_planes(m.wn[0].res, pr);
    pr.taps = c.wn_kernel; pr.seq_len = Tt;
    chain_wn_t = chain_wn_t && gemm_uses_planes(m.wn[0].in_gate, pr);
  }
  float* const hnt_f = chain_t ? nullptr : w.hn;
  void* const hnt_p = chain_t ? w.hn_p : nullptr;
  auto ada_rows = [&](const float* x, const float* g, int mod_idx, int rows, bool planes) {
    RowsNormArgs n;
    n.x_in = x; n.ld_in = D; n.y = planes ? nullptr : w.hn; n.y_planes = planes ? w.hn_p : nullptr; n.ld_y = D; n.M = rows; n.d = D;
    n.mode = NORM_ADA_RMS; n.eps = c.norm_eps; n.g1 = g;
    n.mod_a = mods + (size_t)mod_idx * 2 * D; n.mod_b = n.mod_a + D; n.ld_mod = 0; n.rows_per_batch = 0;
    return rows_norm_forward(n, st);
  };
  auto ada = [&](const float* x, const float* g, int mod_idx) { return ada_rows(x, g, mod_idx, M, chain); };
  if (lag_event && depth < 2) IDX_HIP(hipEventRecord(lag_event, st));
  bool h_compact = false;
  if (gemm(m.merge, w.x_in, Win, w.ha, D, M, st)) return 1;
  float* h = w.ha;
  int pushed = 0;
  for (int i = 0; i < depth; ++i) {
    DiTBlock& B = m.blocks[i];
    if (i > half) {
      float* skip = w.skips[--pushed];
      void* skip_p = chain ? w.skips_p[pushed] : nullptr;
      if (gemm(B.skip_a, h, D, w.hmid, D, M, st, ACT_NONE, nullptr, 0, chain ? w.h_p : nullptr)) return 1;
      float* dst = (h == w.ha) ? w.hb : w.ha;
      if (gemm(B.skip_b, skip, D, dst, D, M, st, ACT_NONE, w.hmid, D, skip_p)) return 1;
      h = dst;
    }
    if (ada(h, B.attn_g, 2 * i)) return 1;
    bool qkv_planes = false;
    {
      GemmArgs g;
      g.x = chain ? nullptr : w.hn; g.x_planes = hn_p; g.ldx = D; g.y = w.qkv; g.ldy = 3 * D; g.M = M;
      const bool fuse_rope = gemm_uses_planes(B.wqkv, g);
      qkv_planes = fuse_rope && D == 64 * c.num_heads;
      if (fuse_rope) { g.rope = m.rope; g.rope_T = T; g.rope_cols = 2 * D; }
      if (qkv_planes) { g.y = nullptr; g.y_planes = w.qkv; }
      if (gemm_forward(B.wqkv, g, st)) return 1;
      if (!fuse_rope && rotary_qk(w.qkv, M, c.num_heads, T, m.rope, st)) return 1;
    }
    AttnPlanesArgs ap;
    ap.planes = w.qkv; ap.Mrows = M; ap.ncols = 3 * D; ap.q_col = 0; ap.k_col = D; ap.v_col = 2 * D; ap.T = T; ap.q_row0 = 0; ap.Sq = T;
    ap.B = N2; ap.H = c.num_heads; ap.kend = w.lens2; ap.scale = 0.125f; ap.o = w.att; ap.o_bs = (long)T * D; ap.o_ts = D;
    AttnArgs a;
    a.q = w.qkv; a.k = w.qkv + D; a.v = w.qkv + 2 * D; a.o = w.att;
    a.q_bs = a.k_bs = a.v_bs = (long)T * 3 * D; a.o_bs = (long)T * D;
    a.q_ts = a.k_ts = a.v_ts = 3 * D; a.o_ts = D;
    a.B = N2; a.H = c.num_heads; a.Sq = T; a.Sk = T; a.causal = 0; a.kend = w.lens2; a.scale = 0.125f;
    a.split_bf16 = get_gemm_mode() == GEMM_BF16X3;
    if (i == depth - 1 && t0 > 0 && i >= half) {
      a.q = w.qkv + (size_t)t0 * 3 * D; a.Sq = Tt; a.o_bs = (long)Tt * D;
      ap.q_row0 = t0; ap.Sq = Tt; ap.o_bs = (long)Tt * D;
      if (chain_t) { a.o = nullptr; a.o_planes = w.att_p; ap.o = nullptr; ap.o_planes = w.att_p; }
      if (qkv_planes ? flash_attn_planes_forward(ap, st) : flash_attn_forward(a, st)) return 1;
      if (gather_tail_rows(w.xres, D, h, D, D, N2, T, t0, st)) return 1;
      if (gemm(B.wo, w.att, D, w.hmid, D, Mt, st, ACT_NONE, w.xres, D, chain_t ? w.att_p : nullptr)) return 1;
      if (ada_rows(w.hmid, B.ffn_g, 2 * i + 1, Mt, chain_t)) return 1;
      if (gemm(B.w13, w.hn, D, chain_t ? nullptr : w.ff, m.ffn, Mt, st, ACT_SWIGLU, nullptr, 0, hnt_p, chain_t ? w.ff_p : nullptr)) return 1;
      float* dst = (h == w.ha) ? w.hb : w.ha;
      if (gemm(B.w2, w.ff, m.ffn, dst, D, Mt, st, ACT_NONE, w.hmid, D, chain_t ? w.ff_p : nullptr, nullptr)) return 1;
      h = dst;
      h_compact = true;
      break;
    }
    if (chain) { a.o = nullptr; a.o_planes = w.att_p; ap.o = nullptr; ap.o_planes = w.att_p; }
    if (qkv_planes ? flash_attn_planes_forward(ap, st) : flash_attn_forward(a, st)) return 1;
    if (i == 0 && lag_event) IDX_HIP(hipEventRecord(lag_event, st));
    if (gemm(B.wo, w.att, D, w.hmid, D, M, st, ACT_NONE, h, D, chain ? w.att_p : nullptr)) return 1;
    if (ada(w.hmid, B.ffn_g, 2 * i + 1)) return 1;
    if (gemm(B.w13, w.hn, D, chain ? nullptr : w.ff, m.ffn, M, st, ACT_SWIGLU, nullptr, 0, hn_p, chain ? w.ff_p : nullptr)) return 1;
    float* dst = (i < half) ? w.skips[pushed] : ((h == w.ha) ? w.hb : w.ha);
    void* dst_p = !chain ? nullptr : (i < half ? w.skips_p[pushed] : (i + 1 < depth && i + 1 > half ? w.h_p : nullptr));
    if (gemm(B.w2, w.ff, m.ffn, dst, D, M, st, ACT_NONE, w.hmid, D, chain ? w.ff_p : nullptr, dst_p)) return 1;
    if (i < half) ++pushed;
    h = dst;
  }
  const float* ht = h;
  const float* xin_t = w.x_in;
  int ld_xin = Win;
  const int* lens_t = w.lens2;
  if (t0 > 0) {
    if (!h_compact) {
      float* hc = (h == w.ha) ? w.hb : w.ha;
      if (gather_tail_rows(hc, D, h, D, D, N2, T, t0, st)) return 1;
      ht = hc;
    }
    if (gather_tail_rows(w.qkv, C, w.x_in, Win, C, N2, T, t0, st)) return 1;
    xin_t = w.qkv; ld_xin = C; lens_t = w.lens2t;
  }
  {
    RowsNormArgs n;
    n.x_in = ht; n.ld_in = D; n.y = hnt_f; n.y_planes = hnt_p; n.ld_y = D; n.M = Mt; n.d = D; n.mode = NORM_ADA_RMS; n.eps = c.norm_eps; n.g1 = m.final_g;
    n.mod_a = mods + (size_t)(2 * depth) * 2 * D; n.mod_b = n.mod_a + D; n.ld_mod = 0; n.rows_per_batch = 0;
    if (rows_norm_forward(n, st)) return 1;
  }
  if (gemm(m.skiplin_a, w.hn, D, w.hmid, D, Mt, st, ACT_NONE, nullptr, 0, hnt_p)) return 1;
  if (gemm(m.skiplin_b, xin_t, ld_xin, w.xres, D, Mt, st, ACT_NONE, w.hmid, D, nullptr, chain_wn_t ? w.xres_p : nullptr)) return 1;
  if (gemm(m.conv1, w.xres, D, w.wn_x, Wh, Mt, st, ACT_NONE, nullptr, 0, chain_wn_t ? w.xres_p : nullptr, chain_wn_t ? w.wnx_p : nullptr)) return 1;
  const int L = c.wn_layers, k = c.wn_kernel;
  for (int l = 0; l < L; ++l) {
    WNLayer& W = m.wn[l];
    int dil = 1;
    for (int q = 0; q < l; ++q) dil *= c.wn_dilation_rate;
    LinearWeights in = W.in_gate;
    in.bias = w.wnb + ((size_t)step * L + l) * 2 * Wh;
    GemmArgs g;
    g.x = chain_wn_t ? nullptr : w.wn_x; g.x_planes = chain_wn_t ? w.wnx_p : nullptr; g.ldx = Wh; g.y = chain_t ? nullptr : w.wn_acts; g.y_planes = chain_t ? w.acts_p : nullptr; g.ldy = Wh; g.M = Mt; g.act = ACT_GATE;
    g.taps = k; g.seq_len = Tt; g.dil = dil; g.pad_left = (k - 1) / 2 * dil; g.pad_mode = 1; g.row_len = lens_t;
    if (gemm_forward(in, g, st)) return 1;
    if (W.has_res) {
      GemmArgs r;
      r.x = chain_t ? nullptr : w.wn_acts; r.x_planes = chain_t ? w.acts_p : nullptr; r.ldx = Wh; r.y = w.wn_x; r.y_planes = chain_wn_t ? w.wnx_p : nullptr; r.ldy = Wh; r.res = w.wn_x; r.ldr = Wh; r.M = Mt; r.seq_len = Tt; r.row_len = lens_t;
      if (gemm_forward(W.res, r, st)) return 1;
    }
    GemmArgs sk;
    sk.x = chain_t ? nullptr : w.wn_acts; sk.x_planes = chain_t ? w.acts_p : nullptr; sk.ldx = Wh; sk.y = w.wn_out; sk.ldy = Wh; sk.M = Mt;
    if (l > 0) { sk.res = w.wn_out; sk.ldr = Wh; }
    if (l == L - 1) { sk.seq_len = Tt; sk.row_len = lens_t; }
    if (gemm_forward(W.skip, sk, st)) return 1;
  }
  if (gemm(m.res_proj, w.xres, D, w.hmid, Wh, Mt, st, ACT_NONE, w.wn_out, Wh, chain_wn_t ? w.xres_p : nullptr)) return 1;
  {
    RowsNormArgs n;
    n.x_in = w.hmid; n.ld_in = Wh; n.y = hnt_f; n.y_planes = hnt_p; n.ld_y = Wh; n.M = Mt; n.d = Wh; n.mode = NORM_MOD_LN; n.eps = 1e-6f;
    n.mod_a = w.fmod + (size_t)step * 2 * Wh; n.mod_b = n.mod_a + Wh; n.ld_mod = 0; n.rows_per_batch = 0;
    if (rows_norm_forward(n, st)) return 1;
  }
  if (gemm(m.final_lin, w.hn, Wh, w.att, Wh, Mt, st, ACT_NONE, nullptr, 0, hnt_p)) return 1;
  return gemm(m.conv2, w.att, Wh, w.vout, C, Mt, st);
}

struct HalfStreams { hipStream_t side = nullptr; hipEvent_t fork = nullptr, lag = nullptr, join = nullptr; };
static std::map<std::pair<int, hipStream_t>, HalfStreams> g_half_streams;
static std::mutex g_half_mu;
static int g_s2mel_overlap = 0;
void set_s2mel_overlap(int on) { g_s2mel_overlap = on ? 1 : 0; }
int get_s2mel_overlap() { return g_s2mel_overlap; }

static int half_streams_for(hipStream_t st, HalfStreams* out) {
  int dev = 0;
  IDX_HIP(hipGetDevice(&dev));
  std::lock_guard<std::mutex> lk(g_half_mu);
  HalfStreams& hs = g_half_streams[std::make_pair(dev, st)];
  if (!hs.side) {
    int prio = 0;
    if (st) IDX_HIP(hipStreamGetPriority(st, &prio));
    IDX_HIP(hipStreamCreateWithPriority(&hs.side, hipStreamNonBlocking, prio));
    IDX_HIP(hipEventCreateWithFlags(&hs.fork, hipEventDisableTiming));
    IDX_HIP(hipEventCreateWithFlags(&hs.lag, hipEventDisableTiming));
    IDX_HIP(hipEventCreateWithFlags(&hs.join, hipEventDisableTiming));
  }
  *out = hs;
  return 0;
}

int s2mel_release_stream(hipStream_t st) {
  int dev = 0;
  IDX_HIP(hipGetDevice(&dev));
  HalfStreams hs;
  {
    std::lock_guard<std::mutex> lk(g_half_mu);
    auto it = g_half_streams.find(std::make_pair(dev, st));
    if (it == g_half_streams.end()) return 0;
    hs = it->second;
    g_half_streams.erase(it);
  }
  if (hs.side) { (void)hipStreamSynchronize(hs.side); (void)hipStreamDestroy(hs.side); }
  if (hs.fork) (void)hipEventDestroy(hs.fork);
  if (hs.lag) (void)hipEventDestroy(hs.lag);
  if (hs.join) (void)hipEventDestroy(hs.join);
  return 0;
}

static bool halves_on_two_streams(hipStream_t st) {
  hipStreamCaptureStatus cap = hipStreamCaptureStatusNone;
  (void)hipStreamIsCapturing(st, &cap);
  return g_s2mel_overlap && !prof_enabled() && cap == hipStreamCaptureStatusNone;
}

static int dit_eval_halves(S2MelModel& m, CfmBuffers& w, int B, int T, int step, bool two_streams, hipStream_t st) {
  if (!two_streams) return dit_eval(m, w, 2 * B, T, step, st, nullptr);
  CfmBuffers v0 = half_view(m, w, 0, B, T);
  CfmBuffers v1 = half_view(m, w, 1, B, T);
  HalfStreams hs;
  if (half_streams_for(st, &hs)) return 1;
  IDX_HIP(hipEventRecord(hs.fork, st));
  IDX_HIP(hipStreamWaitEvent(hs.side, hs.fork, 0));
  if (dit_eval(m, v0, B, T, step, st, hs.lag)) return 1;
  IDX_HIP(hipStreamWaitEvent(hs.side, hs.lag, 0));
  if (dit_eval(m, v1, B, T, step, hs.side, nullptr)) return 1;
  IDX_HIP(hipEventRecord(hs.join, hs.side));
  IDX_HIP(hipStreamWaitEvent(st, hs.join, 0));
  return 0;
}

int S2MelModel::cfm(const float* mu, const int* x_lens_host, const float* prompt, const int* prompt_lens_host, int Tp_max,
                    const float* style, const float* z, const float* t_emb, const float* dt_host, int n_steps, float cfg_rate,
                    float* out, int B, int T, void* ws, size_t ws_bytes, hipStream_t st) {
  IDX_CHECK(mu && x_lens_host && prompt && prompt_lens_host && style && z && t_emb && dt_host && out, "null pointer");
  IDX_CHECK(B > 0 && T > 0 && n_steps > 0 && Tp_max > 0, "shape");
  IDX_CHECK(cfg_rate > 0.0f, "the stacked-CFG path needs inference_cfg_rate > 0 (reference default 0.7)");
  IDX_CHECK(T <= rope_len, "sequence longer than the rope cache");
  IDX_CHECK(ws && ws_bytes >= cfm_workspace_bytes(B, T, n_steps), "workspace too small");
  CfmBuffers w = carve_cfm(*this, ws, B, T, n_steps);
  if (cfm_solve(w, mu, x_lens_host, prompt, prompt_lens_host, Tp_max, style, z, t_emb, dt_host, n_steps, cfg_rate, B, T, st)) return 1;
  IDX_HIP(hipMemcpyAsync(out, w.xstate, (size_t)B * cfg.in_channels * T * sizeof(float), hipMemcpyDeviceToDevice, st));
  return 0;
}

int S2MelModel::cfm_solve(CfmBuffers& w, const float* mu, const int* x_lens_host, const float* prompt, const int* prompt_lens_host,
                          int Tp_max, const float* style, const float* z, const float* t_emb, const float* dt_host, int n_steps,
                          float cfg_rate, int B, int T, hipStream_t st) {
  const int D = cfg.hidden_dim, C = cfg.in_channels, Wh = cfg.wn_hidden, depth = cfg.depth, L = cfg.wn_layers;
  std::vector<int> lens2(2 * B), plen(B);
  for (int b = 0; b < B; ++b) {
    IDX_CHECK(x_lens_host[b] > 0 && x_lens_host[b] <= T && prompt_lens_host[b] >= 0 && prompt_lens_host[b] <= std::min(Tp_max, x_lens_host[b]), "lengths");
    lens2[b] = lens2[B + b] = x_lens_host[b];
    plen[b] = prompt_lens_host[b];
  }
  {
    int halo = 0, dil = 1, pmin = plen[0];
    for (int l = 0; l < L; ++l) { halo += (cfg.wn_kernel - 1) / 2 * dil; dil *= cfg.wn_dilation_rate; }
    for (int b = 0; b < B; ++b) pmin = std::min(pmin, plen[b]);
    w.tail_t0 = pmin - halo >= 64 ? pmin - halo : 0;
  }
  std::vector<int> lens2t(2 * B);
  for (int i = 0; i < 2 * B; ++i) lens2t[i] = lens2[i] - w.tail_t0;
  IDX_HIP(hipMemcpyAsync(w.lens2, lens2.data(), 2 * B * sizeof(int), hipMemcpyHostToDevice, st));
  IDX_HIP(hipMemcpyAsync(w.lens2t, lens2t.data(), 2 * B * sizeof(int), hipMemcpyHostToDevice, st));
  IDX_HIP(hipMemcpyAsync(w.plen, plen.data(), B * sizeof(int), hipMemcpyHostToDevice, st));
  IDX_HIP(hipStreamSynchronize(st));
  if (gemm(temb0, t_emb, 256, w.tmp_steps, D, n_steps, st, ACT_SILU) || gemm(temb2, w.tmp_steps, D, w.t1, D, n_steps, st)) return 1;
  if (gemm(mod_all, w.t1, D, w.mods, (2 * depth + 1) * 2 * D, n_steps, st)) return 1;
  if (silu_rows(w.t1s, w.t1, (size_t)n_steps * D, st) || gemm(final_mod, w.t1s, Wh, w.fmod, 2 * Wh, n_steps, st)) return 1;
  if (gemm(t2emb0, t_emb, 256, w.tmp_steps, Wh, n_steps, st, ACT_SILU) || gemm(t2emb2, w.tmp_steps, Wh, w.t2, Wh, n_steps, st)) return 1;
  if (gemm(wn_cond, w.t2, Wh, w.wnb, L * 2 * Wh, n_steps, st)) return 1;
  if (gemm(cond_proj, mu, cfg.content_dim, w.condp, D, B * T, st)) return 1;
  if (cfm_init_state(w.xstate, z, w.plen, B, C, T, st)) return 1;
  const bool two_streams = halves_on_two_streams(st);
  for (int s = 0; s < n_steps; ++s) {
    CfmPackArgs pk;
    pk.x_in = w.x_in; pk.ld = 2 * C + D + cfg.style_dim; pk.x = w.xstate; pk.prompt = prompt; pk.prompt_len = w.plen;
    pk.cond = w.condp; pk.cond_null = cond_proj.bias; pk.style = style;
    pk.B = B; pk.T = T; pk.C = C; pk.D = D; pk.S = cfg.style_dim; pk.Tp_max = Tp_max;
    pk.x_only = s > 0;
    if (cfm_pack(pk, st)) return 1;
    if (dit_eval_halves(*this, w, B, T, s, two_streams, st)) return 1;
    CfmEulerArgs eu;
    eu.x = w.xstate; eu.v = w.vout; eu.v_null = two_streams ? w.vout + (size_t)B * T * C : nullptr; eu.ldv = C; eu.prompt_len = w.plen; eu.B = B; eu.T = T; eu.C = C; eu.dt = dt_host[s]; eu.cfg_rate = cfg_rate;
    eu.v_t0 = w.tail_t0; eu.v_T = T - w.tail_t0;
    if (cfm_euler(eu, st)) return 1;
  }
  return 0;
}

struct CfmRowsBuffers { float *mu, *prompt; const float **pcond, **ref_mel; int* gen_len; size_t bytes; };

static CfmRowsBuffers carve_cfm_rows(const S2MelModel& m, void* ws, size_t base, int B, int T, int Tp_max) {
  const auto& c = m.cfg;
  CfmRowsBuffers b;
  Carver k(ws ? static_cast<char*>(ws) + base : nullptr);
  b.mu = k.take<float>((size_t)B * T * c.content_dim);
  b.prompt = k.take<float>((size_t)B * c.in_channels * Tp_max);
  b.pcond = k.take<const float*>(B);
  b.ref_mel = k.take<const float*>(B);
  b.gen_len = k.take<int>(B);
  b.bytes = base + ((k.off + 255) & ~(size_t)255);
  return b;
}

size_t S2MelModel::cfm_rows_workspace_bytes(int B, int T, int Tp_max, int n_steps) const {
  return carve_cfm_rows(*this, nullptr, cfm_workspace_bytes(B, T, n_steps), B, T, Tp_max).bytes;
}

int S2MelModel::cfm_rows(const float* gen_cond, const int* target_lens_host, int Tg_max, const float* const* prompt_cond_host,
                         const float* const* ref_mel_host, const int* prompt_lens_host, const float* style, const float* z,
                         const float* t_emb, const float* dt_host, int n_steps, float cfg_rate, float* out, int B, int T, void* ws,
                         size_t ws_bytes, hipStream_t st) {
  IDX_CHECK(gen_cond && target_lens_host && prompt_cond_host && ref_mel_host && prompt_lens_host && style && z && t_emb && dt_host && out,
            "null pointer");
  IDX_CHECK(B > 0 && T > 0 && Tg_max > 0 && n_steps > 0, "shape");
  IDX_CHECK(cfg_rate > 0.0f, "the stacked-CFG path needs inference_cfg_rate > 0 (reference default 0.7)");
  IDX_CHECK(T <= rope_len, "sequence longer than the rope cache");
  IDX_CHECK(cfg.content_dim % 4 == 0 && ((uintptr_t)gen_cond & 15) == 0, "gen_cond must be 16-byte aligned (content_dim % 4 == 0)");
  std::vector<int> xl(B), tg(B);
  int Tp_max = 0, T_need = 0;
  for (int b = 0; b < B; ++b) {
    const int Tp = prompt_lens_host[b], Tg = target_lens_host[b];
    IDX_CHECK(Tp > 0 && Tg > 0 && Tg <= Tg_max, "prompt_lens / target_lens out of range");
    IDX_CHECK(prompt_cond_host[b] && ref_mel_host[b], "null prompt table entry");
    IDX_CHECK(((uintptr_t)prompt_cond_host[b] & 15) == 0, "prompt_condition rows must be 16-byte aligned");
    xl[b] = Tp + Tg;
    tg[b] = Tg;
    Tp_max = std::max(Tp_max, Tp);
    T_need = std::max(T_need, Tp + Tg);
  }
  IDX_CHECK(T == T_need, "T must be max_b(prompt_lens[b] + target_lens[b])");
  IDX_CHECK(ws && ws_bytes >= cfm_rows_workspace_bytes(B, T, Tp_max, n_steps), "workspace too small");
  CfmBuffers w = carve_cfm(*this, ws, B, T, n_steps);
  CfmRowsBuffers r = carve_cfm_rows(*this, ws, w.bytes, B, T, Tp_max);
  IDX_HIP(hipMemcpyAsync(r.pcond, prompt_cond_host, B * sizeof(float*), hipMemcpyHostToDevice, st));
  IDX_HIP(hipMemcpyAsync(r.ref_mel, ref_mel_host, B * sizeof(float*), hipMemcpyHostToDevice, st));
  IDX_HIP(hipMemcpyAsync(r.gen_len, tg.data(), B * sizeof(int), hipMemcpyHostToDevice, st));
  IDX_HIP(hipMemcpyAsync(w.plen, prompt_lens_host, B * sizeof(int), hipMemcpyHostToDevice, st));
  CfmRowsPackArgs pk;
  pk.mu = r.mu; pk.prompt = r.prompt; pk.pcond = r.pcond; pk.ref_mel = r.ref_mel; pk.gen = gen_cond; pk.prompt_len = w.plen;
  pk.gen_len = r.gen_len; pk.B = B; pk.T = T; pk.Dc = cfg.content_dim; pk.C = cfg.in_channels; pk.Tp_max = Tp_max; pk.Tg_max = Tg_max;
  if (cfm_rows_pack(pk, st)) return 1;
  if (cfm_solve(w, r.mu, xl.data(), r.prompt, prompt_lens_host, Tp_max, style, z, t_emb, dt_host, n_steps, cfg_rate, B, T, st)) return 1;
  return cfm_rows_emit(out, w.xstate, w.plen, r.gen_len, B, cfg.in_channels, T, Tg_max, st);
}

int S2MelModel::estimator(const float* x, const float* prompt, const int* prompt_lens_host, int Tp_max, const int* x_lens_host,
                          const float* t_emb, const float* style, const float* mu, float* out_tm, int B, int T, void* ws, size_t ws_bytes,
                          hipStream_t st) {
  IDX_CHECK(x && prompt && prompt_lens_host && x_lens_host && t_emb && style && mu && out_tm, "null pointer");
  IDX_CHECK(B > 0 && T > 0 && Tp_max > 0 && T <= rope_len, "shape");
  IDX_CHECK(ws && ws_bytes >= cfm_workspace_bytes(B, T, 1), "workspace too small");
  const int D = cfg.hidden_dim, C = cfg.in_channels, Wh = cfg.wn_hidden, depth = cfg.depth, L = cfg.wn_layers;
  CfmBuffers w = carve_cfm(*this, ws, B, T, 1);
  std::vector<int> lens2(2 * B), plen(B);
  for (int b = 0; b < B; ++b) {
    IDX_CHECK(x_lens_host[b] > 0 && x_lens_host[b] <= T && prompt_lens_host[b] >= 0 && prompt_lens_host[b] <= std::min(Tp_max, T), "lengths");
    lens2[b] = lens2[B + b] = x_lens_host[b];
    plen[b] = prompt_lens_host[b];
  }
  IDX_HIP(hipMemcpyAsync(w.lens2, lens2.data(), 2 * B * sizeof(int), hipMemcpyHostToDevice, st));
  IDX_HIP(hipMemcpyAsync(w.plen, plen.data(), B * sizeof(int), hipMemcpyHostToDevice, st));
  IDX_HIP(hipStreamSynchronize(st));
  if (gemm(temb0, t_emb, 256, w.tmp_steps, D, 1, st, ACT_SILU) || gemm(temb2, w.tmp_steps, D, w.t1, D, 1, st)) return 1;
  if (gemm(mod_all, w.t1, D, w.mods, (2 * depth + 1) * 2 * D, 1, st)) return 1;
  if (silu_rows(w.t1s, w.t1, (size_t)D, st) || gemm(final_mod, w.t1s, Wh, w.fmod, 2 * Wh, 1, st)) return 1;
  if (gemm(t2emb0, t_emb, 256, w.tmp_steps, Wh, 1, st, ACT_SILU) || gemm(t2emb2, w.tmp_steps, Wh, w.t2, Wh, 1, st)) return 1;
  if (gemm(wn_cond, w.t2, Wh, w.wnb, L * 2 * Wh, 1, st)) return 1;
  if (gemm(cond_proj, mu, cfg.content_dim, w.condp, D, B * T, st)) return 1;
  IDX_HIP(hipMemcpyAsync(w.xstate, x, (size_t)B * C * T * sizeof(float), hipMemcpyDeviceToDevice, st));
  CfmPackArgs pk;
  pk.x_in = w.x_in; pk.ld = 2 * C + D + cfg.style_dim; pk.x = w.xstate; pk.prompt = prompt; pk.prompt_len = w.plen;
  pk.cond = w.condp; pk.cond_null = cond_proj.bias; pk.style = style;
  pk.B = B; pk.T = T; pk.C = C; pk.D = D; pk.S = cfg.style_dim; pk.Tp_max = Tp_max;
  if (cfm_pack(pk, st)) return 1;
  {
    CfmBuffers v0 = half_view(*this, w, 0, B, T);
    if (dit_eval(*this, v0, B, T, 0, st, nullptr)) return 1;
  }
  IDX_HIP(hipMemcpyAsync(out_tm, w.vout, (size_t)B * T * C * sizeof(float), hipMemcpyDeviceToDevice, st));
  return 0;
}


static CondBuffers carve_cond(const S2MelModel& m, void* ws, int B, int M, int Tg) {
  const auto& c = m.cfg;
  CondBuffers b;
  Carver k(ws);
  const size_t rows = (size_t)B * std::max(M, Tg);
  const int wide = std::max(std::max(c.codec_hidden, c.lr_channels), std::max(c.gpt_layer_dims[0], c.gpt_layer_dims[1]));
  b.a = k.take<float>(rows * wide);
  b.b = k.take<float>(rows * wide);
  b.s = k.take<float>(rows * wide);
  b.stats = k.take<float>(2 * B);
  b.idx_code = k.take<int>((size_t)B * M);
  b.idx_row = k.take<int>((size_t)B * M);
  b.idx_interp = k.take<int>((size_t)B * Tg);
  b.tlen = k.take<int>(B);
  b.bytes = (k.off + 255) & ~(size_t)255;
  return b;
}

size_t S2MelModel::cond_workspace_bytes(int B, int M, int Tg) const { return carve_cond(*this, nullptr, B, M, Tg).bytes; }

int S2MelModel::prepare_cond(const float* latent, const long long* codes, const int* code_lens_host, const int* target_lens_host,
                             int B, int M, int Tg, float* cond_out, void* ws, size_t ws_bytes, hipStream_t st) {
  IDX_CHECK(latent && codes && code_lens_host && target_lens_host && cond_out, "null pointer");
  IDX_CHECK(B > 0 && M > 0 && Tg > 0, "shape");
  IDX_CHECK(ws && ws_bytes >= cond_workspace_bytes(B, M, Tg), "workspace too small");
  const int Hc = cfg.codec_hidden;
  CondBuffers w = carve_cond(*this, ws, B, M, Tg);
  std::vector<long long> hc((size_t)B * M);
  IDX_HIP(hipMemcpyAsync(hc.data(), codes, hc.size() * sizeof(long long), hipMemcpyDeviceToHost, st));
  IDX_HIP(hipStreamSynchronize(st));
  std::vector<int> ic((size_t)B * M), ir((size_t)B * M), ii((size_t)B * Tg, -1), tl(B);
  for (int b = 0; b < B; ++b) {
    const int mb = code_lens_host[b], tb = target_lens_host[b];
    IDX_CHECK(mb > 0 && mb <= M && tb > 0 && tb <= Tg, "code_lens / target_lens out of range");
    tl[b] = tb;
    for (int i = 0; i < M; ++i) {
      const long long cde = hc[(size_t)b * M + i];
      IDX_CHECK(i >= mb || (cde >= 0 && cde < cfg.codebook_size), "semantic code out of the codebook");
      ic[(size_t)b * M + i] = i < mb ? (int)cde : -1;
      ir[(size_t)b * M + i] = i < mb ? b * M + i : -1;
    }
    const float scale = (float)mb / (float)tb;
    for (int j = 0; j < tb; ++j) ii[(size_t)b * Tg + j] = b * M + std::min((int)std::floor((float)j * scale), mb - 1);
  }
  IDX_HIP(hipMemcpyAsync(w.idx_code, ic.data(), ic.size() * sizeof(int), hipMemcpyHostToDevice, st));
  IDX_HIP(hipMemcpyAsync(w.idx_row, ir.data(), ir.size() * sizeof(int), hipMemcpyHostToDevice, st));
  IDX_HIP(hipMemcpyAsync(w.idx_interp, ii.data(), ii.size() * sizeof(int), hipMemcpyHostToDevice, st));
  IDX_HIP(hipMemcpyAsync(w.tlen, tl.data(), B * sizeof(int), hipMemcpyHostToDevice, st));
  IDX_HIP(hipStreamSynchronize(st));
  const int rowsM = B * M;
  if (gemm(gl[0], latent, cfg.gpt_dim, w.a, gl[0].N, rowsM, st) || gemm(gl[1], w.a, gl[0].N, w.b, gl[1].N, rowsM, st) ||
      gemm(gl[2], w.b, gl[1].N, w.a, Hc, rowsM, st)) return 1;
  GatherArgs ga;
  ga.out = w.s; ga.ld_out = Hc; ga.d = Hc;
  ga.table[0] = vq_table; ga.idx[0] = w.idx_code;
  ga.table[1] = w.a; ga.idx[1] = w.idx_row;
  if (gather_sum_rows(ga, rowsM, st)) return 1;
  return regulate_rows(w.s, w, B, M, Tg, cond_out, st);
}

int S2MelModel::regulate_rows(const float* s_rows, const CondBuffers& w, int B, int M, int Tg, float* cond_out, hipStream_t st) {
  const int Hc = cfg.codec_hidden, LC = cfg.lr_channels;
  const int rowsM = B * M, rowsT = B * Tg;
  if (gemm(lr_in, s_rows, Hc, w.a, LC, rowsM, st)) return 1;
  GatherArgs gi;
  gi.out = w.b; gi.ld_out = LC; gi.d = LC; gi.table[0] = w.a; gi.idx[0] = w.idx_interp;
  if (gather_sum_rows(gi, rowsT, st)) return 1;
  float* cur = w.b;
  float* other = w.a;
  for (int n = 0; n < cfg.lr_num_convs; ++n) {
    GemmArgs g;
    g.x = cur; g.ldx = LC; g.y = other; g.ldy = LC; g.M = rowsT; g.taps = 3; g.seq_len = Tg; g.dil = 1; g.pad_left = 1; g.pad_mode = 0;
    if (gemm_forward(lr_conv[n], g, st)) return 1;
    if (groupnorm1_mish(cur, other, lr_gn_g[n], lr_gn_b[n], w.tlen, B, Tg, LC, 1e-5f, w.stats, st)) return 1;
  }
  GemmArgs o;
  o.x = cur; o.ldx = LC; o.y = cond_out; o.ldy = LC; o.M = rowsT; o.seq_len = Tg; o.row_len = w.tlen;
  return gemm_forward(lr_out, o, st);
}

int S2MelModel::regulate(const float* S, const int* in_lens_host, const int* target_lens_host, int B, int M, int Tg, float* cond_out,
                         void* ws, size_t ws_bytes, hipStream_t st) {
  IDX_CHECK(S && in_lens_host && target_lens_host && cond_out, "null pointer");
  IDX_CHECK(B > 0 && M > 0 && Tg > 0, "shape");
  IDX_CHECK(ws && ws_bytes >= cond_workspace_bytes(B, M, Tg), "workspace too small");
  CondBuffers w = carve_cond(*this, ws, B, M, Tg);
  std::vector<int> ii((size_t)B * Tg, -1), tl(B);
  for (int b = 0; b < B; ++b) {
    const int mb = in_lens_host[b], tb = target_lens_host[b];
    IDX_CHECK(mb > 0 && mb <= M && tb > 0 && tb <= Tg, "in_lens / target_lens out of range");
    tl[b] = tb;
    const float scale = (float)mb / (float)tb;
    for (int j = 0; j < tb; ++j) ii[(size_t)b * Tg + j] = b * M + std::min((int)std::floor((float)j * scale), mb - 1);
  }
  IDX_HIP(hipMemcpyAsync(w.idx_interp, ii.data(), ii.size() * sizeof(int), hipMemcpyHostToDevice, st));
  IDX_HIP(hipMemcpyAsync(w.tlen, tl.data(), B * sizeof(int), hipMemcpyHostToDevice, st));
  IDX_HIP(hipStreamSynchronize(st));
  return regulate_rows(S, w, B, M, Tg, cond_out, st);
}

}
```

Measured before the change: 186.9.

## Add 16x16x32 MFMA variant of bf16x3 GEMM and route s2mel linears to it

Measured after the change: 189.4 (median of 6 runs). +1.4%, better.

```diff
diff --git a/index-tts_amd/csrc/capi.hip b/index-tts_amd/csrc/capi.hip
--- a/index-tts_amd/csrc/capi.hip
+++ b/index-tts_amd/csrc/capi.hip
@@ -232,7 +232,7 @@
   std::vector<float> hw, hb;
   if (fetch(weight, (size_t)N * K, &hw)) return 1;
   if (bias && fetch(bias, N, &hb)) return 1;
-  if (make_linear(l->arena, hw.data(), bias ? hb.data() : nullptr, N, K, {WP16_ALWAYS, weight_is_kn ? W_KN : W_NK}, &l->w)) return 1;
+  if (make_linear(l->arena, hw.data(), bias ? hb.data() : nullptr, N, K, {WP16_ALWAYS_MF16, weight_is_kn ? W_KN : W_NK}, &l->w)) return 1;
   *out = l.release();
   return 0;
   API_END
@@ -244,7 +244,10 @@
   IDX_CHECK(lin, "null handle");
   GemmArgs a;
   a.x = x; a.ldx = ldx; a.y = y; a.ldy = ldy; a.res = residual; a.ldr = ldr; a.M = M; a.act = act;
-  return bf16x3 ? gemm_bf16x3_forward(lin->w, a, static_cast<hipStream_t>(stream)) : gemm_tn_forward(lin->w, a, static_cast<hipStream_t>(stream));
+  if (!bf16x3) return gemm_tn_forward(lin->w, a, static_cast<hipStream_t>(stream));
+  LinearWeights w = lin->w;
+  if (bf16x3 == 2) w.mf16 = false;
+  return gemm_bf16x3_forward(w, a, static_cast<hipStream_t>(stream));
   API_END
 }
 
diff --git a/index-tts_amd/csrc/gemm.h b/index-tts_amd/csrc/gemm.h
--- a/index-tts_amd/csrc/gemm.h
+++ b/index-tts_amd/csrc/gemm.h
@@ -11,6 +11,7 @@
   const float* bias = nullptr;
   int N = 0, K = 0;
   const void* wp16 = nullptr;
+  bool mf16 = false;
 };
 
 static inline size_t linear_packed_floats(int N, int K) { return (size_t)cdiv(N, 32) * cdiv(K, 16) * 512; }
diff --git a/index-tts_amd/csrc/gemm_bf16x3_v2.hip b/index-tts_amd/csrc/gemm_bf16x3_v2.hip
--- a/index-tts_amd/csrc/gemm_bf16x3_v2.hip
+++ b/index-tts_amd/csrc/gemm_bf16x3_v2.hip
@@ -70,12 +70,13 @@
 
 #define V2_WAITCNT(vm) __builtin_amdgcn_s_waitcnt(((vm) & 15) | (((vm) >> 4) << 14) | 0x70)
 
-template <bool TAPS, int EPI, int CFG>
+template <bool TAPS, int EPI, int MF>
 __device__ __forceinline__ void gemm_v2_tile(const GemmV2P& q, const int bm, const int bn, const int tid) {
-  constexpr int NSTAGE = CFG ? 3 : 4;
-  constexpr int WMW = CFG ? 2 : 4, WNW = 2, TN = CFG ? 2 : 4;
+  constexpr int NSTAGE = 3;
+  constexpr int WMW = 2, WNW = 2, TN = 2;
   constexpr int BM = 64 * WMW, BN = 32 * TN * WNW;
   static_assert(BM / 32 == WMW * WNW && BN / 32 == WMW * WNW, "one 32-row block of A and of B per wave and plane");
+  static_assert(MF == 32 || MF == 16, "MFMA shape");
   constexpr int PLANE = BM * 32;
   constexpr int STAGE_BYTES = 4 * PLANE;
   constexpr int PPW = 4;
@@ -130,118 +131,218 @@
     }
   };
 
-  const int sw = (h ^ ((j >> 3) & 1)) * 16;
-  const int a_off = (wm * 64 + j) * 32 + sw;
-  const int b_offr = (wn * TN * 32 + j) * 32 + sw;
-
-  f32x16 acc[2][TN];
-#pragma unroll
-  for (int a = 0; a < 2; ++a)
-#pragma unroll
-    for (int b = 0; b < TN; ++b)
-#pragma unroll
-      for (int r = 0; r < 16; ++r) acc[a][b][r] = 0.0f;
-
-  for (int s = 0; s < NSTAGE; ++s)
-    if (s < ns) {
-#pragma unroll
-      for (int pi = 0; pi < PPW; ++pi) issue_piece(pi);
-      advance();
+  if constexpr (MF == 16) {
+    const int g = lane >> 4, r16 = lane & 15;
+    const int sw = ((g & 1) ^ ((r16 >> 3) & 1)) * 16;
+    const int a_off = (wm * 64 + r16) * 32 + sw;
+    const int b_off = 2 * PLANE + (wn * 64 + r16) * 32 + sw;
+    f32x4 acc[4][4];
+#pragma unroll
+    for (int a = 0; a < 4; ++a)
+#pragma unroll
+      for (int b = 0; b < 4; ++b)
+#pragma unroll
+        for (int r = 0; r < 4; ++r) acc[a][b][r] = 0.0f;
+    for (int s = 0; s < NSTAGE; ++s)
+      if (s < ns) {
+#pragma unroll
+        for (int pi = 0; pi < PPW; ++pi) issue_piece(pi);
+        advance();
+      }
+
+    typedef unsigned u32x4 __attribute__((ext_vector_type(4)));
+    auto pair_step = [&](const bool tail, const bool vm_one_behind, const int nreq) {
+      if (vm_one_behind) V2_WAITCNT(PPW); else V2_WAITCNT(0);
+      __builtin_amdgcn_s_barrier();
+      __builtin_amdgcn_sched_barrier(0);
+      const int second = rslot + 1 == NSTAGE ? 0 : rslot + 1;
+      const char* st = smv2 + ((g >> 1) && !tail ? second : rslot) * STAGE_BYTES;
+      rslot = second + 1 == NSTAGE ? 0 : second + 1;
+      bf16x8 ah[4], al[4], bh[4], bl[4];
+      auto rd_a = [&](int t) {
+        ah[t] = *reinterpret_cast<const bf16x8*>(st + a_off + t * 512);
+        al[t] = *reinterpret_cast<const bf16x8*>(st + PLANE + a_off + t * 512);
+      };
+      auto rd_b = [&](int t) {
+        bh[t] = *reinterpret_cast<const bf16x8*>(st + b_off + t * 512);
+        bl[t] = *reinterpret_cast<const bf16x8*>(st + PLANE + b_off + t * 512);
+      };
+      rd_a(0); rd_b(0);
+      __builtin_amdgcn_sched_barrier(0);
+      rd_a(1);
+      __builtin_amdgcn_sched_barrier(0);
+      rd_a(2);
+      __builtin_amdgcn_sched_barrier(0);
+      rd_a(3);
+      __builtin_amdgcn_sched_barrier(0);
+#pragma unroll
+      for (int t = 1; t < 4; ++t) rd_b(t);
+      if (tail) {
+        const unsigned keep = (g >> 1) ? 0u : 0xffffffffu;
+#pragma unroll
+        for (int t = 0; t < 4; ++t) {
+          ah[t] = (bf16x8)((u32x4)ah[t] & keep); al[t] = (bf16x8)((u32x4)al[t] & keep);
+          bh[t] = (bf16x8)((u32x4)bh[t] & keep); bl[t] = (bf16x8)((u32x4)bl[t] & keep);
+        }
+      }
+#define V2_MFMA3(nt)                                                                                               \
+      _Pragma("unroll") for (int mt = 0; mt < 4; ++mt) {                                                            \
+        acc[mt][nt] = __builtin_amdgcn_mfma_f32_16x16x32_bf16(al[mt], bh[nt], acc[mt][nt], 0, 0, 0);                \
+        acc[mt][nt] = __builtin_amdgcn_mfma_f32_16x16x32_bf16(ah[mt], bl[nt], acc[mt][nt], 0, 0, 0);                \
+        acc[mt][nt] = __builtin_amdgcn_mfma_f32_16x16x32_bf16(ah[mt], bh[nt], acc[mt][nt], 0, 0, 0);                \
+      }
+#define V2_MFMA1(mt, nt)                                                                                           \
+      acc[mt][nt] = __builtin_amdgcn_mfma_f32_16x16x32_bf16(al[mt], bh[nt], acc[mt][nt], 0, 0, 0);                  \
+      acc[mt][nt] = __builtin_amdgcn_mfma_f32_16x16x32_bf16(ah[mt], bl[nt], acc[mt][nt], 0, 0, 0);                  \
+      acc[mt][nt] = __builtin_amdgcn_mfma_f32_16x16x32_bf16(ah[mt], bh[nt], acc[mt][nt], 0, 0, 0);                  \
+      __builtin_amdgcn_sched_barrier(0);
+
+      __builtin_amdgcn_sched_barrier(0);
+      V2_MFMA1(0, 0) V2_MFMA1(1, 0) V2_MFMA1(2, 0) V2_MFMA1(3, 0)
+      V2_WAITCNT(63);
+      __builtin_amdgcn_s_barrier();
+      __builtin_amdgcn_sched_barrier(0);
+      if (nreq >= 1) { issue_piece(0); issue_piece(1); }
+      __builtin_amdgcn_sched_barrier(0);
+      V2_MFMA3(1)
+      __builtin_amdgcn_sched_barrier(0);
+      if (nreq >= 1) { issue_piece(2); issue_piece(3); advance(); }
+      if (nreq >= 2) { issue_piece(0); issue_piece(1); }
+      __builtin_amdgcn_sched_barrier(0);
+      V2_MFMA3(2)
+      __builtin_amdgcn_sched_barrier(0);
+      if (nreq >= 2) { issue_piece(2); issue_piece(3); advance(); }
+      __builtin_amdgcn_sched_barrier(0);
+      V2_MFMA3(3)
+      __builtin_amdgcn_sched_barrier(0);
+#undef V2_MFMA1
+#undef V2_MFMA3
+    };
+    V2_STAMP(1);
+    int done = 0;
+    for (; ist + 2 <= ns && ist > done + 2; done += 2) pair_step(false, true, 2);
+    for (; done + 2 <= ns; done += 2) pair_step(false, ist > done + 2, min(ns - ist, 2));
+    if (done < ns) pair_step(true, false, 0);
+    V2_STAMP(2);
+    auto write_pass = [&](int ps, float* lds, int RS) {
+#pragma unroll
+      for (int nt = 0; nt < 4; ++nt)
+#pragma unroll
+        for (int e = 0; e < 4; ++e) lds[(4 * g + e) * RS + nt * 16 + r16] = acc[ps][nt][e];
+    };
+    gemm_epilogue_wave<EPI, TN, 3>(p, write_pass, reinterpret_cast<float*>(smv2), bm * BM + wm * 64, bn * BN + wn * TN * 32, wave, lane);
+  } else {
+    const int sw = (h ^ ((j >> 3) & 1)) * 16;
+    const int a_off = (wm * 64 + j) * 32 + sw;
+    const int b_offr = (wn * TN * 32 + j) * 32 + sw;
+
+    f32x16 acc[2][TN];
+#pragma unroll
+    for (int a = 0; a < 2; ++a)
+#pragma unroll
+      for (int b = 0; b < TN; ++b)
+#pragma unroll
+        for (int r = 0; r < 16; ++r) acc[a][b][r] = 0.0f;
+
+    for (int s = 0; s < NSTAGE; ++s)
+      if (s < ns) {
+#pragma unroll
+        for (int pi = 0; pi < PPW; ++pi) issue_piece(pi);
+        advance();
+      }
+
+    struct Frag { bf16x8 ah[2], al[2], bh[TN], bl[TN]; };
+    auto wait_stage = [&](int s) {
+      const int rem = ns - 1 - s;
+      if (rem >= 1) V2_WAITCNT(PPW);
+      else V2_WAITCNT(0);
+      __builtin_amdgcn_s_barrier();
+      __builtin_amdgcn_sched_barrier(0);
+    };
+    auto load_frags = [&](Frag& f) {
+      const char* st = smv2 + rslot * STAGE_BYTES;
+      rslot = rslot + 1 == NSTAGE ? 0 : rslot + 1;
+#pragma unroll
+      for (int t = 0; t < 2; ++t) {
+        f.ah[t] = *reinterpret_cast<const bf16x8*>(st + a_off + t * 1024);
+        f.al[t] = *reinterpret_cast<const bf16x8*>(st + PLANE + a_off + t * 1024);
+      }
+#pragma unroll
+      for (int t = 0; t < TN; ++t) {
+        f.bh[t] = *reinterpret_cast<const bf16x8*>(st + 2 * PLANE + b_offr + t * 1024);
+        f.bl[t] = *reinterpret_cast<const bf16x8*>(st + 3 * PLANE + b_offr + t * 1024);
+      }
+    };
+    auto compute = [&](const Frag& f, const bool more) {
+#define V2_MFMA3(mt, nt)                                                                                         \
+      acc[mt][nt] = __builtin_amdgcn_mfma_f32_32x32x16_bf16(f.al[mt], f.bh[nt], acc[mt][nt], 0, 0, 0);             \
+      acc[mt][nt] = __builtin_amdgcn_mfma_f32_32x32x16_bf16(f.ah[mt], f.bl[nt], acc[mt][nt], 0, 0, 0);             \
+      acc[mt][nt] = __builtin_amdgcn_mfma_f32_32x32x16_bf16(f.ah[mt], f.bh[nt], acc[mt][nt], 0, 0, 0);
+      V2_MFMA3(0, 0)
+      __builtin_amdgcn_sched_barrier(0);
+      if (more) issue_piece(0);
+      __builtin_amdgcn_sched_barrier(0);
+      V2_MFMA3(0, 1)
+      __builtin_amdgcn_sched_barrier(0);
+      if (more) issue_piece(1);
+      __builtin_amdgcn_sched_barrier(0);
+      V2_MFMA3(1, 0)
+      __builtin_amdgcn_sched_barrier(0);
+      if (more) issue_piece(2);
+      __builtin_amdgcn_sched_barrier(0);
+      V2_MFMA3(1, 1)
+      __builtin_amdgcn_sched_barrier(0);
+      if (more) { issue_piece(3); advance(); }
+      __builtin_amdgcn_sched_barrier(0);
+#undef V2_MFMA3
+    };
+
+    Frag f0, f1;
+    {
+      const int rem = ns - 1;
+      if (rem >= 2) V2_WAITCNT(2 * PPW);
+      else if (rem >= 1) V2_WAITCNT(PPW);
+      else V2_WAITCNT(0);
+      __builtin_amdgcn_s_barrier();
+      __builtin_amdgcn_sched_barrier(0);
     }
-
-  struct Frag { bf16x8 ah[2], al[2], bh[TN], bl[TN]; };
-  auto wait_stage = [&](int s) {
-    const int rem = ns - 1 - s;
-    if (NSTAGE >= 4 && rem >= 2) V2_WAITCNT(2 * PPW);
-    else if (NSTAGE >= 3 && rem >= 1) V2_WAITCNT(PPW);
-    else V2_WAITCNT(0);
-    __builtin_amdgcn_s_barrier();
-    __builtin_amdgcn_sched_barrier(0);
-  };
-  auto load_frags = [&](Frag& f) {
-    const char* st = smv2 + rslot * STAGE_BYTES;
-    rslot = rslot + 1 == NSTAGE ? 0 : rslot + 1;
-#pragma unroll
-    for (int t = 0; t < 2; ++t) {
-      f.ah[t] = *reinterpret_cast<const bf16x8*>(st + a_off + t * 1024);
-      f.al[t] = *reinterpret_cast<const bf16x8*>(st + PLANE + a_off + t * 1024);
+    V2_STAMP(1);
+    load_frags(f0);
+    int i = 0;
+    for (; i + NSTAGE + 1 < ns; i += 2) {
+      V2_WAITCNT((NSTAGE - 2) * PPW);
+      __builtin_amdgcn_s_barrier();
+      __builtin_amdgcn_sched_barrier(0);
+      load_frags(f1);
+      compute(f0, true);
+      V2_WAITCNT((NSTAGE - 2) * PPW);
+      __builtin_amdgcn_s_barrier();
+      __builtin_amdgcn_sched_barrier(0);
+      load_frags(f0);
+      compute(f1, true);
     }
-#pragma unroll
-    for (int t = 0; t < TN; ++t) {
-      f.bh[t] = *reinterpret_cast<const bf16x8*>(st + 2 * PLANE + b_offr + t * 1024);
-      f.bl[t] = *reinterpret_cast<const bf16x8*>(st + 3 * PLANE + b_offr + t * 1024);
+    for (; i < ns; i += 2) {
+      if (i + 1 < ns) { wait_stage(i + 1); load_frags(f1); }
+      else V2_WAITCNT(0);
+      compute(f0, ist < ns);
+      if (i + 1 < ns) {
+        if (i + 2 < ns) { wait_stage(i + 2); load_frags(f0); }
+        else V2_WAITCNT(0);
+        compute(f1, ist < ns);
+      }
     }
-  };
-  auto compute = [&](const Frag& f, const bool more) {
-#define V2_MFMA3(mt, nt)                                                                                         \
-    acc[mt][nt] = __builtin_amdgcn_mfma_f32_32x32x16_bf16(f.al[mt], f.bh[nt], acc[mt][nt], 0, 0, 0);             \
-    acc[mt][nt] = __builtin_amdgcn_mfma_f32_32x32x16_bf16(f.ah[mt], f.bl[nt], acc[mt][nt], 0, 0, 0);             \
-    acc[mt][nt] = __builtin_amdgcn_mfma_f32_32x32x16_bf16(f.ah[mt], f.bh[nt], acc[mt][nt], 0, 0, 0);
-    if constexpr (TN == 4) { V2_MFMA3(0, 0) V2_MFMA3(0, 1) } else { V2_MFMA3(0, 0) }
-    __builtin_amdgcn_sched_barrier(0);
-    if (more) issue_piece(0);
-    __builtin_amdgcn_sched_barrier(0);
-    if constexpr (TN == 4) { V2_MFMA3(0, 2) V2_MFMA3(0, 3) } else { V2_MFMA3(0, 1) }
-    __builtin_amdgcn_sched_barrier(0);
-    if (more) issue_piece(1);
-    __builtin_amdgcn_sched_barrier(0);
-    if constexpr (TN == 4) { V2_MFMA3(1, 0) V2_MFMA3(1, 1) } else { V2_MFMA3(1, 0) }
-    __builtin_amdgcn_sched_barrier(0);
-    if (more) issue_piece(2);
-    __builtin_amdgcn_sched_barrier(0);
-    if constexpr (TN == 4) { V2_MFMA3(1, 2) V2_MFMA3(1, 3) } else { V2_MFMA3(1, 1) }
-    __builtin_amdgcn_sched_barrier(0);
-    if (more) { issue_piece(3); advance(); }
-    __builtin_amdgcn_sched_barrier(0);
-#undef V2_MFMA3
-  };
-
-  Frag f0, f1;
-  {
-    const int rem = ns - 1;
-    if (NSTAGE >= 4 && rem >= 3) V2_WAITCNT(3 * PPW);
-    else if (NSTAGE >= 3 && rem >= 2) V2_WAITCNT(2 * PPW);
-    else if (rem >= 1) V2_WAITCNT(PPW);
-    else V2_WAITCNT(0);
-    __builtin_amdgcn_s_barrier();
-    __builtin_amdgcn_sched_barrier(0);
-  }
-  V2_STAMP(1);
-  load_frags(f0);
-  int i = 0;
-  for (; i + NSTAGE + 1 < ns; i += 2) {
-    V2_WAITCNT((NSTAGE - 2) * PPW);
-    __builtin_amdgcn_s_barrier();
-    __builtin_amdgcn_sched_barrier(0);
-    load_frags(f1);
-    compute(f0, true);
-    V2_WAITCNT((NSTAGE - 2) * PPW);
-    __builtin_amdgcn_s_barrier();
-    __builtin_amdgcn_sched_barrier(0);
-    load_frags(f0);
-    compute(f1, true);
-  }
-  for (; i < ns; i += 2) {
-    if (i + 1 < ns) { wait_stage(i + 1); load_frags(f1); }
-    else V2_WAITCNT(0);
-    compute(f0, ist < ns);
-    if (i + 1 < ns) {
-      if (i + 2 < ns) { wait_stage(i + 2); load_frags(f0); }
-      else V2_WAITCNT(0);
-      compute(f1, ist < ns);
-    }
-  }
-  V2_STAMP(2);
-  auto write_pass = [&](int ps, float* lds, int RS) {
-    const int mt = ps >> 1, hh = ps & 1;
-#pragma unroll
-    for (int nt = 0; nt < TN; ++nt)
-#pragma unroll
-      for (int qq = 0; qq < 2; ++qq)
-#pragma unroll
-        for (int e = 0; e < 4; ++e) lds[(8 * qq + 4 * h + e) * RS + nt * 32 + j] = acc[mt][nt][(2 * hh + qq) * 4 + e];
-  };
-  gemm_epilogue_wave<EPI, TN, 3>(p, write_pass, reinterpret_cast<float*>(smv2), bm * BM + wm * 64, bn * BN + wn * TN * 32, wave, lane);
+    V2_STAMP(2);
+    auto write_pass = [&](int ps, float* lds, int RS) {
+      const int mt = ps >> 1, hh = ps & 1;
+#pragma unroll
+      for (int nt = 0; nt < TN; ++nt)
+#pragma unroll
+        for (int qq = 0; qq < 2; ++qq)
+#pragma unroll
+          for (int e = 0; e < 4; ++e) lds[(8 * qq + 4 * h + e) * RS + nt * 32 + j] = acc[mt][nt][(2 * hh + qq) * 4 + e];
+    };
+    gemm_epilogue_wave<EPI, TN, 3>(p, write_pass, reinterpret_cast<float*>(smv2), bm * BM + wm * 64, bn * BN + wn * TN * 32, wave, lane);
+  }
   V2_STAMP(6);
 #ifdef V2_TIMING
   asm volatile("s_waitcnt vmcnt(0)" ::: "memory");
@@ -249,8 +350,8 @@
   V2_STAMP(3); V2_RSTAMP(5);
 }
 
-template <bool TAPS, int EPI, int CFG>
-__global__ __launch_bounds__(CFG ? 256 : 512, CFG ? 3 : 2) void gemm_bf16x3_v2_kernel(const GemmV2P q) {
+template <bool TAPS, int EPI, int MF>
+__global__ __launch_bounds__(256, 3) void gemm_bf16x3_v2_kernel(const GemmV2P q) {
   const GemmKP& p = q.g;
   const int L = blockIdx.x, xcd = L & 7, qq = L >> 3;
   int bn, bm;
@@ -262,7 +363,7 @@
     if (bn >= p.nblocks) return;
   } else { bn = qq / p.mt8; bm = (qq - bn * p.mt8) * 8 + xcd; }
   if (bm >= p.mtiles) return;
-  gemm_v2_tile<TAPS, EPI, CFG>(q, bm, bn, threadIdx.x);
+  gemm_v2_tile<TAPS, EPI, MF>(q, bm, bn, threadIdx.x);
 }
 
 StreamScratch g_plane_scratch(8);
@@ -294,8 +395,7 @@
     IDX_CHECK(a.rope_T > 0 && a.rope_cols % 64 == 0 && a.act == ACT_NONE && (a.ldy & 3) == 0, "fused rotary arguments");
     q.g.rope = a.rope; q.g.rope_T = a.rope_T; q.g.rope_cols = a.rope_cols;
   }
-  const int cfg = 1;
-  const int BMh = cfg ? 128 : 256, BNh = cfg ? 128 : 256;
+  const int BMh = 128, BNh = 128;
   q.g.mtiles = cdiv(a.M, BMh);
   q.g.mt8 = cdiv(q.g.mtiles, 8);
   q.g.nblocks = cdiv(w.N, BNh);
@@ -322,19 +422,23 @@
   IDX_CHECK(grid < (1ll << 31), "grid size");
   static const int cat = prof_register("gemm_bf16x3_v2_kernel");
   ProfScope prof(cat, stream, flops, bytes);
-  const int lds = cfg ? 3 * (4 * 128 * 32) : 4 * (4 * 256 * 32);
+  const int lds = 3 * (4 * 128 * 32);
   const bool paired = a.act == ACT_SWIGLU || a.act == ACT_GATE;
   IDX_CHECK(!(a.rope && (a.res || paired)), "the rotary epilogue takes no residual and no paired activation");
   IDX_CHECK(!a.row_len || a.seq_len >= 16, "row masks need seq_len >= 16");
   const int epi = a.rope ? EPI_ROPE : paired ? EPI_PAIRED : a.act != ACT_NONE ? EPI_ACT : EPI_PLAIN;
   typedef void (*KernelFn)(const GemmV2P);
-#define V2_ROW(T, C) gemm_bf16x3_v2_kernel<T, EPI_PLAIN, C>, gemm_bf16x3_v2_kernel<T, EPI_ROPE, C>, gemm_bf16x3_v2_kernel<T, EPI_PAIRED, C>, gemm_bf16x3_v2_kernel<T, EPI_ACT, C>
-  static const KernelFn kernels[2][2][4] = {{{V2_ROW(false, 0)}, {V2_ROW(true, 0)}}, {{V2_ROW(false, 1)}, {V2_ROW(true, 1)}}};
-  static DynLdsLimit lds_limit[2];
-  IDX_HIP(lds_limit[0].set(4 * (4 * 256 * 32), V2_ROW(false, 0), V2_ROW(true, 0)));
-  IDX_HIP(lds_limit[1].set(3 * (4 * 128 * 32), V2_ROW(false, 1), V2_ROW(true, 1)));
+#define V2_ROW(T, F) gemm_bf16x3_v2_kernel<T, EPI_PLAIN, F>, gemm_bf16x3_v2_kernel<T, EPI_ROPE, F>, gemm_bf16x3_v2_kernel<T, EPI_PAIRED, F>, gemm_bf16x3_v2_kernel<T, EPI_ACT, F>
+  static const KernelFn kernels[2][2][4] = {{{V2_ROW(false, 32)}, {V2_ROW(true, 32)}}, {{V2_ROW(false, 16)}, {V2_ROW(true, 16)}}};
+  static DynLdsLimit lds_limit;
+  IDX_HIP(lds_limit.set(lds, V2_ROW(false, 32), V2_ROW(true, 32), V2_ROW(false, 16), V2_ROW(true, 16)));
+  int mf16 = w.mf16 ? 1 : 0;
+#ifdef V2_EXP_SHAPE
+  if (const char* e = getenv("IDXTTS_EXP_V2_SHAPE")) mf16 = atoi(e) == 16;
+#endif
+  const KernelFn kernel = kernels[mf16][a.taps > 1 ? 1 : 0][epi];
 #undef V2_ROW
-  hipLaunchKernelGGL(kernels[cfg][a.taps > 1 ? 1 : 0][epi], dim3((unsigned)grid), dim3(cfg ? 256 : 512), lds, stream, q);
+  hipLaunchKernelGGL(kernel, dim3((unsigned)grid), dim3(256), lds, stream, q);
   IDX_LAUNCH_CHECK();
   return 0;
 }
diff --git a/index-tts_amd/csrc/model_util.h b/index-tts_amd/csrc/model_util.h
--- a/index-tts_amd/csrc/model_util.h
+++ b/index-tts_amd/csrc/model_util.h
@@ -17,6 +17,7 @@
 enum Wp16Policy {
   WP16_ALWAYS,
   WP16_DMA_SHAPES,
+  WP16_ALWAYS_MF16,
 };
 enum WeightLayout { W_NK , W_KN  };
 struct LinearOpts {
diff --git a/index-tts_amd/csrc/model_util.hip b/index-tts_amd/csrc/model_util.hip
--- a/index-tts_amd/csrc/model_util.hip
+++ b/index-tts_amd/csrc/model_util.hip
@@ -55,7 +55,8 @@
   pack_linear(packed.data(), w, N, Kpad);
   if (up(arena, packed, &out->wp)) return 1;
   out->N = N; out->K = Kpad;
-  if (o.wp16 == WP16_ALWAYS || (N >= 96 && Kpad % 16 == 0)) {
+  out->mf16 = o.wp16 == WP16_ALWAYS_MF16;
+  if (o.wp16 != WP16_DMA_SHAPES || (N >= 96 && Kpad % 16 == 0)) {
     std::vector<float> p16((linear_bf16x3_packed_bytes(N, Kpad) + 3) / 4);
     pack_linear_bf16x3(p16.data(), w, N, Kpad);
     const float* d16 = nullptr;
diff --git a/index-tts_amd/csrc/s2mel.hip b/index-tts_amd/csrc/s2mel.hip
--- a/index-tts_amd/csrc/s2mel.hip
+++ b/index-tts_amd/csrc/s2mel.hip
@@ -68,12 +68,12 @@
   for (int i = 0; i < depth; ++i) {
     DiTBlock& B = blocks[i];
     const std::string p = e + ".transformer.layers." + std::to_string(i);
-    if (linear_from(t, arena, p + ".attention.wqkv", 3 * D, D, false, WP16_ALWAYS, &B.wqkv)) return 1;
-    if (linear_from(t, arena, p + ".attention.wo", D, D, false, WP16_ALWAYS, &B.wo)) return 1;
+    if (linear_from(t, arena, p + ".attention.wqkv", 3 * D, D, false, WP16_ALWAYS_MF16, &B.wqkv)) return 1;
+    if (linear_from(t, arena, p + ".attention.wo", D, D, false, WP16_ALWAYS_MF16, &B.wo)) return 1;
     HostTensor *w1 = nullptr, *w3 = nullptr;
     if (need(t, p + ".feed_forward.w1.weight", {ffn, D}, &w1) || need(t, p + ".feed_forward.w3.weight", {ffn, D}, &w3)) return 1;
-    if (make_linear(arena, pair_pack(w1->data.data(), w3->data.data(), ffn, D).data(), nullptr, 2 * ffn, D, {WP16_ALWAYS}, &B.w13)) return 1;
-    if (linear_from(t, arena, p + ".feed_forward.w2", D, ffn, false, WP16_ALWAYS, &B.w2)) return 1;
+    if (make_linear(arena, pair_pack(w1->data.data(), w3->data.data(), ffn, D).data(), nullptr, 2 * ffn, D, {WP16_ALWAYS_MF16}, &B.w13)) return 1;
+    if (linear_from(t, arena, p + ".feed_forward.w2", D, ffn, false, WP16_ALWAYS_MF16, &B.w2)) return 1;
     HostTensor *g = nullptr;
     if (need(t, p + ".attention_norm.norm.weight", {D}, &g) || up(arena, g->data, &B.attn_g)) return 1;
     if (need(t, p + ".ffn_norm.norm.weight", {D}, &g) || up(arena, g->data, &B.ffn_g)) return 1;
@@ -81,35 +81,35 @@
     if (i > depth / 2) {
       HostTensor *sw = nullptr, *sb = nullptr;
       if (need(t, p + ".skip_in_linear.weight", {D, 2 * D}, &sw) || need(t, p + ".skip_in_linear.bias", {D}, &sb)) return 1;
-      if (make_linear(arena, col_slice(sw->data, D, 2 * D, 0, D).data(), sb->data.data(), D, D, {WP16_ALWAYS}, &B.skip_a)) return 1;
-      if (make_linear(arena, col_slice(sw->data, D, 2 * D, D, 2 * D).data(), nullptr, D, D, {WP16_ALWAYS}, &B.skip_b)) return 1;
+      if (make_linear(arena, col_slice(sw->data, D, 2 * D, 0, D).data(), sb->data.data(), D, D, {WP16_ALWAYS_MF16}, &B.skip_a)) return 1;
+      if (make_linear(arena, col_slice(sw->data, D, 2 * D, D, 2 * D).data(), nullptr, D, D, {WP16_ALWAYS_MF16}, &B.skip_b)) return 1;
     }
   }
   {
     HostTensor* g = nullptr;
     if (need(t, e + ".transformer.norm.norm.weight", {D}, &g) || up(arena, g->data, &final_g)) return 1;
     if (append_mod(e + ".transformer.norm")) return 1;
-    if (make_linear(arena, mod_w.data(), mod_b.data(), (2 * depth + 1) * 2 * D, D, {WP16_ALWAYS}, &mod_all)) return 1;
+    if (make_linear(arena, mod_w.data(), mod_b.data(), (2 * depth + 1) * 2 * D, D, {WP16_ALWAYS_MF16}, &mod_all)) return 1;
   }
   const int Win = 2 * C + D + cfg.style_dim;
-  if (linear_from(t, arena, e + ".cond_projection", D, cfg.content_dim, true, WP16_ALWAYS, &cond_proj)) return 1;
-  if (linear_from(t, arena, e + ".cond_x_merge_linear", D, Win, true, WP16_ALWAYS, &merge)) return 1;
-  if (linear_from(t, arena, e + ".t_embedder.mlp.0", D, 256, true, WP16_ALWAYS, &temb0) || linear_from(t, arena, e + ".t_embedder.mlp.2", D, D, true, WP16_ALWAYS, &temb2)) return 1;
-  if (linear_from(t, arena, e + ".t_embedder2.mlp.0", Wh, 256, true, WP16_ALWAYS, &t2emb0) || linear_from(t, arena, e + ".t_embedder2.mlp.2", Wh, Wh, true, WP16_ALWAYS, &t2emb2)) return 1;
+  if (linear_from(t, arena, e + ".cond_projection", D, cfg.content_dim, true, WP16_ALWAYS_MF16, &cond_proj)) return 1;
+  if (linear_from(t, arena, e + ".cond_x_merge_linear", D, Win, true, WP16_ALWAYS_MF16, &merge)) return 1;
+  if (linear_from(t, arena, e + ".t_embedder.mlp.0", D, 256, true, WP16_ALWAYS_MF16, &temb0) || linear_from(t, arena, e + ".t_embedder.mlp.2", D, D, true, WP16_ALWAYS_MF16, &temb2)) return 1;
+  if (linear_from(t, arena, e + ".t_embedder2.mlp.0", Wh, 256, true, WP16_ALWAYS_MF16, &t2emb0) || linear_from(t, arena, e + ".t_embedder2.mlp.2", Wh, Wh, true, WP16_ALWAYS_MF16, &t2emb2)) return 1;
   {
     HostTensor *sw = nullptr, *sb = nullptr;
     if (need(t, e + ".skip_linear.weight", {D, D + C}, &sw) || need(t, e + ".skip_linear.bias", {D}, &sb)) return 1;
-    if (make_linear(arena, col_slice(sw->data, D, D + C, 0, D).data(), sb->data.data(), D, D, {WP16_ALWAYS}, &skiplin_a)) return 1;
-    if (make_linear(arena, col_slice(sw->data, D, D + C, D, D + C).data(), nullptr, D, C, {WP16_ALWAYS}, &skiplin_b)) return 1;
-  }
-  if (linear_from(t, arena, e + ".conv1", Wh, D, true, WP16_ALWAYS, &conv1)) return 1;
-  if (linear_from(t, arena, e + ".res_projection", Wh, D, true, WP16_ALWAYS, &res_proj)) return 1;
-  if (linear_from(t, arena, e + ".final_layer.linear", Wh, Wh, true, WP16_ALWAYS, &final_lin)) return 1;
-  if (linear_from(t, arena, e + ".final_layer.adaLN_modulation.1", 2 * Wh, Wh, true, WP16_ALWAYS, &final_mod)) return 1;
+    if (make_linear(arena, col_slice(sw->data, D, D + C, 0, D).data(), sb->data.data(), D, D, {WP16_ALWAYS_MF16}, &skiplin_a)) return 1;
+    if (make_linear(arena, col_slice(sw->data, D, D + C, D, D + C).data(), nullptr, D, C, {WP16_ALWAYS_MF16}, &skiplin_b)) return 1;
+  }
+  if (linear_from(t, arena, e + ".conv1", Wh, D, true, WP16_ALWAYS_MF16, &conv1)) return 1;
+  if (linear_from(t, arena, e + ".res_projection", Wh, D, true, WP16_ALWAYS_MF16, &res_proj)) return 1;
+  if (linear_from(t, arena, e + ".final_layer.linear", Wh, Wh, true, WP16_ALWAYS_MF16, &final_lin)) return 1;
+  if (linear_from(t, arena, e + ".final_layer.adaLN_modulation.1", 2 * Wh, Wh, true, WP16_ALWAYS_MF16, &final_mod)) return 1;
   {
     HostTensor *w = nullptr, *b = nullptr;
     if (need(t, e + ".conv2.weight", {C, Wh, 1}, &w) || need(t, e + ".conv2.bias", {C}, &b)) return 1;
-    if (make_linear(arena, w->data.data(), b->data.data(), C, Wh, {WP16_ALWAYS}, &conv2)) return 1;
+    if (make_linear(arena, w->data.data(), b->data.data(), C, Wh, {WP16_ALWAYS_MF16}, &conv2)) return 1;
   }
   const int L = cfg.wn_layers, k = cfg.wn_kernel;
   wn.resize(L);
@@ -124,7 +124,7 @@
       HostTensor *iw = nullptr, *ib = nullptr;
       if (need(t, p + ".weight", {2 * Wh, Wh, k}, &iw) || need(t, p + ".bias", {2 * Wh}, &ib)) return 1;
       const std::vector<float> rows = conv_to_rows(iw->data, 2 * Wh, Wh, k);
-      if (make_linear(arena, pair_pack(rows.data(), rows.data() + (size_t)Wh * k * Wh, Wh, k * Wh).data(), nullptr, 2 * Wh, k * Wh, {WP16_ALWAYS}, &W.in_gate)) return 1;
+      if (make_linear(arena, pair_pack(rows.data(), rows.data() + (size_t)Wh * k * Wh, Wh, k * Wh).data(), nullptr, 2 * Wh, k * Wh, {WP16_ALWAYS_MF16}, &W.in_gate)) return 1;
       const float* cwl = cw->data.data() + (size_t)l * 2 * Wh * Wh;
       const std::vector<float> cwp = pair_pack(cwl, cwl + (size_t)Wh * Wh, Wh, Wh);
       cw_perm.insert(cw_perm.end(), cwp.begin(), cwp.end());
@@ -139,16 +139,16 @@
       if (l < L - 1) {
         std::vector<float> w_res(rw->data.begin(), rw->data.begin() + (size_t)Wh * Wh), b_res(rb->data.begin(), rb->data.begin() + Wh);
         std::vector<float> w_skip(rw->data.begin() + (size_t)Wh * Wh, rw->data.end()), b_skip(rb->data.begin() + Wh, rb->data.end());
-        if (make_linear(arena, w_res.data(), b_res.data(), Wh, Wh, {WP16_ALWAYS}, &W.res) || make_linear(arena, w_skip.data(), b_skip.data(), Wh, Wh, {WP16_ALWAYS}, &W.skip)) return 1;
+        if (make_linear(arena, w_res.data(), b_res.data(), Wh, Wh, {WP16_ALWAYS_MF16}, &W.res) || make_linear(arena, w_skip.data(), b_skip.data(), Wh, Wh, {WP16_ALWAYS_MF16}, &W.skip)) return 1;
       } else {
         W.has_res = false;
-        if (make_linear(arena, rw->data.data(), rb->data.data(), Wh, Wh, {WP16_ALWAYS}, &W.skip)) return 1;
+        if (make_linear(arena, rw->data.data(), rb->data.data(), Wh, Wh, {WP16_ALWAYS_MF16}, &W.skip)) return 1;
       }
     }
-    if (make_linear(arena, cw_perm.data(), cb_perm.data(), 2 * Wh * L, Wh, {WP16_ALWAYS}, &wn_cond)) return 1;
+    if (make_linear(arena, cw_perm.data(), cb_perm.data(), 2 * Wh * L, Wh, {WP16_ALWAYS_MF16}, &wn_cond)) return 1;
   }
   const int LC = cfg.lr_channels;
-  if (linear_from(t, arena, "length_regulator.content_in_proj", LC, cfg.lr_in_channels, true, WP16_ALWAYS, &lr_in)) return 1;
+  if (linear_from(t, arena, "length_regulator.content_in_proj", LC, cfg.lr_in_channels, true, WP16_ALWAYS_MF16, &lr_in)) return 1;
   lr_conv.resize(cfg.lr_num_convs);
   lr_gn_g.resize(cfg.lr_num_convs);
   lr_gn_b.resize(cfg.lr_num_convs);
@@ -156,7 +156,7 @@
     HostTensor *w = nullptr, *b = nullptr, *g = nullptr, *bb = nullptr;
     const std::string p = "length_regulator.model." + std::to_string(3 * n);
     if (need(t, p + ".weight", {LC, LC, 3}, &w) || need(t, p + ".bias", {LC}, &b)) return 1;
-    if (make_linear(arena, conv_to_rows(w->data, LC, LC, 3).data(), b->data.data(), LC, 3 * LC, {WP16_ALWAYS}, &lr_conv[n])) return 1;
+    if (make_linear(arena, conv_to_rows(w->data, LC, LC, 3).data(), b->data.data(), LC, 3 * LC, {WP16_ALWAYS_MF16}, &lr_conv[n])) return 1;
     const std::string q = "length_regulator.model." + std::to_string(3 * n + 1);
     if (need(t, q + ".weight", {LC}, &g) || need(t, q + ".bias", {LC}, &bb)) return 1;
     if (up(arena, g->data, &lr_gn_g[n]) || up(arena, bb->data, &lr_gn_b[n])) return 1;
@@ -165,12 +165,12 @@
     HostTensor *w = nullptr, *b = nullptr;
     const std::string p = "length_regulator.model." + std::to_string(3 * cfg.lr_num_convs);
     if (need(t, p + ".weight", {LC, LC, 1}, &w) || need(t, p + ".bias", {LC}, &b)) return 1;
-    if (make_linear(arena, w->data.data(), b->data.data(), LC, LC, {WP16_ALWAYS}, &lr_out)) return 1;
+    if (make_linear(arena, w->data.data(), b->data.data(), LC, LC, {WP16_ALWAYS_MF16}, &lr_out)) return 1;
   }
   {
     const int dims[4] = {cfg.gpt_dim, cfg.gpt_layer_dims[0], cfg.gpt_layer_dims[1], cfg.gpt_layer_dims[2]};
     for (int n = 0; n < 3; ++n)
-      if (linear_from(t, arena, "gpt_layer." + std::to_string(n), dims[n + 1], dims[n], true, WP16_ALWAYS, &gl[n])) return 1;
+      if (linear_from(t, arena, "gpt_layer." + std::to_string(n), dims[n + 1], dims[n], true, WP16_ALWAYS_MF16, &gl[n])) return 1;
     IDX_CHECK(dims[3] == cfg.codec_hidden && cfg.codec_hidden == cfg.lr_in_channels, "gpt_layer / codec / length-regulator widths");
   }
   {
```
